# FrozenWolf-Cyber/Indic-CL-ASR

Hardware: AMD Instinct MI355X
Metric: utterances/sec (15 s @16 kHz) Conformer-M RNNT-CTC+EWC train step (higher is better)
Workload: dtype bf16; 1 GPU; BASELINE configs[1]: Conformer-medium (d=256, 16L, H=640) hybrid RNNT-CTC + EWC, bs=32/GPU x 15 s, bf16 projections, freeze_encoder_till=12, 22x257 heads, fused_batch_size=4; global_batch=32, parallelism=dp1

## Files before the change

### indic_cl_asr_amd/csrc/attention_flash_bwd.hip

```cpp
#include "attention_flash.h"
#include "partials.h"

namespace {

constexpr int FB_THREADS = 256;
constexpr int FB_ROWB = 128;
constexpr int FB_T64 = 64 * FB_ROWB;
constexpr int FB_PBUF = 128 * FB_ROWB;
constexpr int FB_SR_LD = 104;
constexpr int FB_SB_LD = 120;
constexpr int FB_Q_STRIP = 16 * (FB_SR_LD + FB_SB_LD) * 2;
constexpr int FB_Q_LDS = 2 * FB_T64 + FB_PBUF + 4 * FB_Q_STRIP;
constexpr int FB_S3_LD = 72;
constexpr int FB_KV_STAGE = 3 * FB_T64 + FB_PBUF + 512;
constexpr int FB_KV_LDS = FB_KV_STAGE + 4 * 16 * FB_S3_LD * 2;

struct FbArgs {
    const __bf16* qkv; const __bf16* pl; const float* bias_u; const float* bias_v; const int64_t* lens;
    const __bf16* ctx; const __bf16* dctx; const float* lse;
    __bf16* dqkv; __bf16* dBand; __bf16* QvHM; float* D; float* part;
    int B, T, H, dk, Rs, pad0; float scale; unsigned seed, thr; float keep_scale;
};

__device__ __forceinline__ void fb_lds_fence() {
    __builtin_amdgcn_fence(__ATOMIC_RELEASE, "wavefront");
    __builtin_amdgcn_wave_barrier();
    __builtin_amdgcn_fence(__ATOMIC_ACQUIRE, "wavefront");
}

__device__ __forceinline__ bf8 fb_tr_pair(const unsigned char* tile, int rowA, int rowB, int sl, int half) {
    const s4v lo = __builtin_amdgcn_ds_read_tr16_b64_v4i16(
        (__attribute__((address_space(3))) s4v*)(tile + rowA * FB_ROWB + ((sl ^ (rowA & 7)) * 16) + half * 8));
    const s4v hi = __builtin_amdgcn_ds_read_tr16_b64_v4i16(
        (__attribute__((address_space(3))) s4v*)(tile + rowB * FB_ROWB + ((sl ^ (rowB & 7)) * 16) + half * 8));
    union { s4v s[2]; bf8 v; } f;
    f.s[0] = lo; f.s[1] = hi;
    return f.v;
}

template <bool DK64>
__global__ __launch_bounds__(FB_THREADS, 2) void relpos_flash_bwd_q_kernel(FbArgs a) {
    extern __shared__ __attribute__((aligned(16))) unsigned char smem[];
    const int tid = threadIdx.x, lane = tid & 63, wave = tid >> 6;
    const int c = lane & 15, q4 = lane >> 4;
    const int T = a.T, H = a.H, dk = a.dk, d = H * dk, B = a.B;
    const int nqt = (T + 63) / 64;
    const int xcd = blockIdx.x & 7, slot_id = blockIdx.x >> 3;
    const int bh = xcd + 8 * (slot_id / nqt);
    if (bh >= B * H) return;
    const int qt = slot_id % nqt;
    const int h = bh % H, b = bh / H;
    int len = (int)a.lens[b];
    len = len < 0 ? 0 : (len > T ? T : len);
    const int I0 = qt * 64, iw = I0 + wave * 16, iq = iw + c;
    const int iqc = iq < T ? iq : T - 1;
    const bool qvalid = iq < len;
    float* part_row = a.part + (size_t)(b * nqt + qt) * (2 * d);

    bf8 Qu[2], Qv[2], dOa[2];
    float Drow = 0.f;
    {
        const __bf16* qrow = a.qkv + ((size_t)b * T + iqc) * (3 * d) + h * dk;
        const __bf16* orow = a.ctx + ((size_t)b * T + iqc) * d + h * dk;
        const __bf16* grow = a.dctx + ((size_t)b * T + iqc) * d + h * dk;
#pragma unroll
        for (int ks = 0; ks < 2; ++ks) {
            union { uint4 u; __bf16 e[8]; bf8 v; } q, o, g;
            q.u = fa_load_slot<DK64>(qrow, ks * 4 + q4, dk);
            o.u = fa_load_slot<DK64>(orow, ks * 4 + q4, dk);
            g.u = fa_load_slot<DK64>(grow, ks * 4 + q4, dk);
            dOa[ks] = g.v;
#pragma unroll
            for (int j = 0; j < 8; ++j) {
                const int e = ks * 32 + q4 * 8 + j;
                const float bu = (e < dk) ? a.bias_u[h * dk + e] : 0.f, bv = (e < dk) ? a.bias_v[h * dk + e] : 0.f;
                Qu[ks][j] = (__bf16)((float)q.e[j] + bu);
                Qv[ks][j] = (__bf16)((float)q.e[j] + bv);
                Drow += (float)g.e[j] * (float)o.e[j];
            }
            if (iq < T)
                *reinterpret_cast<bf8*>(a.QvHM + ((size_t)(h * B + b) * T + iq) * 64 + ks * 32 + q4 * 8) = Qv[ks];
        }
        Drow += __shfl_xor(Drow, 16, 64);
        Drow += __shfl_xor(Drow, 32, 64);
        if (!qvalid) Drow = 0.f;
        if (iq < T && q4 == 0) a.D[(size_t)bh * T + iq] = Drow;
    }
    const float lse_i = qvalid ? a.lse[(size_t)bh * T + iq] : 0.f;
    __bf16* dqrow = a.dqkv + ((size_t)b * T + iqc) * (3 * d) + h * dk;
    if (I0 >= len) {
        if (iq < T)
            for (int mt = 0; mt < 4; ++mt)
                if (mt * 16 + q4 * 4 < dk) *reinterpret_cast<uint2*>(dqrow + mt * 16 + q4 * 4) = make_uint2(0, 0);
        if (tid < 2 * dk) part_row[(tid / dk) * d + h * dk + (tid % dk)] = 0.f;
        return;
    }
    const unsigned char* sK = smem;
    const unsigned char* sV = smem + FB_T64;
    const unsigned char* sP = smem + 2 * FB_T64;
    unsigned char* sR = smem + 2 * FB_T64 + FB_PBUF + wave * FB_Q_STRIP;
    unsigned char* sB = sR + 16 * FB_SR_LD * 2;
    for (int i = lane; i < 16 * FB_SB_LD * 2 / 16; i += 64) reinterpret_cast<uint4*>(sB)[i] = make_uint4(0, 0, 0, 0);

    uint4 rk[2], rv[2], rp[4];
    const __bf16* kbase = a.qkv + (size_t)b * T * (3 * d) + d + h * dk;
    const __bf16* vbase = kbase + d;
    const __bf16* pbase = a.pl + h * dk;
#define FBQ_FETCH(t_)                                                                                         \
    do {                                                                                                      \
        const int j0_ = (t_) * 64;                                                                            \
        _Pragma("unroll") for (int i_ = 0; i_ < 2; ++i_) {                                                    \
            const int idx_ = tid + i_ * FB_THREADS, row_ = idx_ >> 3, sl_ = idx_ & 7;                         \
            int j_ = j0_ + row_; j_ = j_ < T ? j_ : T - 1;                                                    \
            rk[i_] = fa_load_slot<DK64>(kbase + (size_t)j_ * (3 * d), sl_, dk);                               \
            rv[i_] = fa_load_slot<DK64>(vbase + (size_t)j_ * (3 * d), sl_, dk);                               \
        }                                                                                                     \
        const int R0_ = T - 1 - I0 - 63 + j0_;                                                                \
        _Pragma("unroll") for (int i_ = 0; i_ < 4; ++i_) {                                                    \
            const int idx_ = tid + i_ * FB_THREADS, row_ = idx_ >> 3, sl_ = idx_ & 7;                         \
            int r_ = R0_ + row_; r_ = r_ < 0 ? 0 : (r_ > 2 * T - 2 ? 2 * T - 2 : r_);                         \
            rp[i_] = fa_load_slot<DK64>(pbase + (size_t)r_ * d, sl_, dk);                                     \
        }                                                                                                     \
    } while (0)
#define FBQ_COMMIT()                                                                                          \
    do {                                                                                                      \
        _Pragma("unroll") for (int i_ = 0; i_ < 2; ++i_) {                                                    \
            const int idx_ = tid + i_ * FB_THREADS, row_ = idx_ >> 3, sl_ = idx_ & 7;                         \
            const int off_ = row_ * FB_ROWB + ((sl_ ^ (row_ & 7)) * 16);                                      \
            *reinterpret_cast<uint4*>(smem + off_) = rk[i_];                                                  \
            *reinterpret_cast<uint4*>(smem + FB_T64 + off_) = rv[i_];                                         \
        }                                                                                                     \
        _Pragma("unroll") for (int i_ = 0; i_ < 4; ++i_) {                                                    \
            const int idx_ = tid + i_ * FB_THREADS, row_ = idx_ >> 3, sl_ = idx_ & 7;                         \
            *reinterpret_cast<uint4*>(smem + 2 * FB_T64 + row_ * FB_ROWB + ((sl_ ^ (row_ & 7)) * 16)) = rp[i_]; \
        }                                                                                                     \
    } while (0)

    const int nkt = (len + 63) / 64;
    FBQ_FETCH(0);
    FBQ_COMMIT();
    __syncthreads();

    f4 dQu[4], dQv[4];
#pragma unroll
    for (int mt = 0; mt < 4; ++mt) { dQu[mt] = (f4){0.f, 0.f, 0.f, 0.f}; dQv[mt] = (f4){0.f, 0.f, 0.f, 0.f}; }
    const int frow = lane >> 2, fch = (lane & 3) * 2;
    __bf16* brow = a.dBand + ((size_t)(h * B + b) * T + (iw + frow < T ? iw + frow : T - 1)) * a.Rs;
    const bool fvalid = iw + frow < T;
    const int pw0 = (3 - wave) * 16;

    for (int t = 0; t < nkt; ++t) {
        if (t + 1 < nkt) FBQ_FETCH(t + 1);
        const int j0 = t * 64;
        {
            f4 R[5];
#pragma unroll
            for (int rt = 0; rt < 5; ++rt) {
                R[rt] = (f4){0.f, 0.f, 0.f, 0.f};
                const int row = pw0 + rt * 16 + c;
#pragma unroll
                for (int ks = 0; ks < 2; ++ks) {
                    const bf8 pf = *reinterpret_cast<const bf8*>(sP + row * FB_ROWB + (((ks * 4 + q4) ^ (row & 7)) * 16));
                    R[rt] = __builtin_amdgcn_mfma_f32_16x16x32_bf16(pf, Qv[ks], R[rt], 0, 0, 0);
                }
            }
#pragma unroll
            for (int rt = 0; rt < 5; ++rt)
#pragma unroll
                for (int r = 0; r < 4; ++r)
                    *reinterpret_cast<__bf16*>(sR + (c * FB_SR_LD + rt * 16 + q4 * 4 + r + c + 1) * 2) = (__bf16)R[rt][r];
        }
        f4 S[4], dP[4];
#pragma unroll
        for (int jt = 0; jt < 4; ++jt) {
            S[jt] = (f4){0.f, 0.f, 0.f, 0.f};
            dP[jt] = (f4){0.f, 0.f, 0.f, 0.f};
            const int row = jt * 16 + c;
#pragma unroll
            for (int ks = 0; ks < 2; ++ks) {
                const int off = row * FB_ROWB + (((ks * 4 + q4) ^ (row & 7)) * 16);
                const bf8 kf = *reinterpret_cast<const bf8*>(sK + off);
                const bf8 vf = *reinterpret_cast<const bf8*>(sV + off);
                S[jt] = __builtin_amdgcn_mfma_f32_16x16x32_bf16(kf, Qu[ks], S[jt], 0, 0, 0);
                dP[jt] = __builtin_amdgcn_mfma_f32_16x16x32_bf16(vf, dOa[ks], dP[jt], 0, 0, 0);
            }
        }
        fb_lds_fence();
        bf8 dSf[2];
#pragma unroll
        for (int jt = 0; jt < 4; ++jt) {
            union { uint2 u; __bf16 e[4]; } bd;
            bd.u = *reinterpret_cast<const uint2*>(sR + (c * FB_SR_LD + jt * 16 + q4 * 4 + 16) * 2);
            unsigned rnd4 = 0;
            if (a.thr > 0) rnd4 = fa_keep_rand4(a.seed, bh, T, iq, (j0 + jt * 16 + q4 * 4) >> 2);
#pragma unroll
            for (int r = 0; r < 4; ++r) {
                const int j = j0 + jt * 16 + q4 * 4 + r;
                const float s = (S[jt][r] + (float)bd.e[r]) * a.scale;
                const float p = (qvalid && j < len) ? __expf(s - lse_i) : 0.f;
                float g = dP[jt][r];
                if (a.thr > 0) g = (((rnd4 >> (8 * r)) & 0xFFu) >= a.thr) ? g * a.keep_scale : 0.f;
                const float ds = p * (g - Drow) * a.scale;
                const __bf16 dsb = (__bf16)ds;
                dSf[jt >> 1][(jt & 1) * 4 + r] = dsb;
                S[jt][r] = (float)dsb;
            }
        }
#pragma unroll
        for (int kk = 0; kk < 2; ++kk)
#pragma unroll
            for (int mt = 0; mt < 4; ++mt) {
                const int qq = c >> 2, p = c & 3;
                const int rowA = kk * 32 + q4 * 4 + qq;
                const bf8 kf = fb_tr_pair(sK, rowA, rowA + 16, mt * 2 + (p >> 1), p & 1);
                dQu[mt] = __builtin_amdgcn_mfma_f32_16x16x32_bf16(kf, dSf[kk], dQu[mt], 0, 0, 0);
            }
        for (int i = lane; i < 16 * 12; i += 64) {
            const int row = i / 12, ch = i - row * 12;
            *reinterpret_cast<uint4*>(sB + (row * FB_SB_LD + ch * 8) * 2) = make_uint4(0, 0, 0, 0);
        }
        fb_lds_fence();
#pragma unroll
        for (int jt = 0; jt < 4; ++jt)
#pragma unroll
            for (int r = 0; r < 4; ++r)
                *reinterpret_cast<__bf16*>(sB + (c * FB_SB_LD + jt * 16 + q4 * 4 + r + 15 - c) * 2) = (__bf16)S[jt][r];
        fb_lds_fence();
#pragma unroll
        for (int kk = 0; kk < 3; ++kk) {
            const bf8 bfrag = *reinterpret_cast<const bf8*>(sB + (c * FB_SB_LD + kk * 32 + q4 * 8) * 2);
#pragma unroll
            for (int mt = 0; mt < 4; ++mt) {
                const int qq = c >> 2, p = c & 3;
                int rowA = pw0 + kk * 32 + q4 * 8 + qq, rowB = rowA + 4;
                rowA = rowA < 127 ? rowA : 127; rowB = rowB < 127 ? rowB : 127;
                const bf8 pf = fb_tr_pair(sP, rowA, rowB, mt * 2 + (p >> 1), p & 1);
                dQv[mt] = __builtin_amdgcn_mfma_f32_16x16x32_bf16(pf, bfrag, dQv[mt], 0, 0, 0);
            }
        }
        {
            uint4 v0 = *reinterpret_cast<const uint4*>(sB + (frow * FB_SB_LD + fch * 8) * 2);
            uint4 v1 = *reinterpret_cast<const uint4*>(sB + (frow * FB_SB_LD + fch * 8 + 8) * 2);
            if ((lane & 3) == 0) {
                const uint4 c0 = *reinterpret_cast<const uint4*>(sB + (frow * FB_SB_LD + 96) * 2);
                const uint4 c1 = *reinterpret_cast<const uint4*>(sB + (frow * FB_SB_LD + 104) * 2);
                v0.x |= c0.x; v0.y |= c0.y; v0.z |= c0.z; v0.w |= c0.w;
                v1.x |= c1.x; v1.y |= c1.y; v1.z |= c1.z; v1.w |= c1.w;
                const uint4 n0 = *reinterpret_cast<const uint4*>(sB + (frow * FB_SB_LD + 64) * 2);
                const uint4 n1 = *reinterpret_cast<const uint4*>(sB + (frow * FB_SB_LD + 72) * 2);
                *reinterpret_cast<uint4*>(sB + (frow * FB_SB_LD + 96) * 2) = n0;
                *reinterpret_cast<uint4*>(sB + (frow * FB_SB_LD + 104) * 2) = n1;
            }
            if (fvalid) {
                const int gcol = T - 16 - iw + j0 + a.pad0 + fch * 8;
                if (gcol >= 0) *reinterpret_cast<uint4*>(brow + gcol) = v0;
                if (gcol + 8 >= 0) *reinterpret_cast<uint4*>(brow + gcol + 8) = v1;
            }
        }
        __syncthreads();
        if (t + 1 < nkt) {
            FBQ_COMMIT();
            __syncthreads();
        }
    }
#undef FBQ_FETCH
#undef FBQ_COMMIT
    fb_lds_fence();
    if ((lane & 3) == 0 && fvalid) {
        const int gcol = T - 16 - iw + (nkt - 1) * 64 + a.pad0 + 64;
        *reinterpret_cast<uint4*>(brow + gcol) = *reinterpret_cast<const uint4*>(sB + (frow * FB_SB_LD + 96) * 2);
        *reinterpret_cast<uint4*>(brow + gcol + 8) = *reinterpret_cast<const uint4*>(sB + (frow * FB_SB_LD + 104) * 2);
    }
    if (iq < T) {
#pragma unroll
        for (int mt = 0; mt < 4; ++mt) {
            if (mt * 16 + q4 * 4 < dk) {
                union { uint2 u; __bf16 e[4]; } o;
#pragma unroll
                for (int r = 0; r < 4; ++r) o.e[r] = (__bf16)(dQu[mt][r] + dQv[mt][r]);
                *reinterpret_cast<uint2*>(dqrow + mt * 16 + q4 * 4) = o.u;
            }
        }
    }
    float* red = reinterpret_cast<float*>(smem);
#pragma unroll
    for (int mt = 0; mt < 4; ++mt)
#pragma unroll
        for (int r = 0; r < 4; ++r) {
            float su = dQu[mt][r], sv = dQv[mt][r];
#pragma unroll
            for (int o = 1; o < 16; o <<= 1) { su += __shfl_xor(su, o, 64); sv += __shfl_xor(sv, o, 64); }
            if (c == 0) {
                red[(wave * 2 + 0) * 64 + mt * 16 + q4 * 4 + r] = su;
                red[(wave * 2 + 1) * 64 + mt * 16 + q4 * 4 + r] = sv;
            }
        }
    __syncthreads();
    if (tid < 2 * dk) {
        const int which = tid / dk, e = tid % dk;
        part_row[which * d + h * dk + e] = (red[(0 * 2 + which) * 64 + e] + red[(1 * 2 + which) * 64 + e]) +
                                           (red[(2 * 2 + which) * 64 + e] + red[(3 * 2 + which) * 64 + e]);
    }
}

template <bool DK64>
__global__ __launch_bounds__(FB_THREADS, 2) void relpos_flash_bwd_kv_kernel(FbArgs a) {
    extern __shared__ __attribute__((aligned(16))) unsigned char smem[];
    const int tid = threadIdx.x, lane = tid & 63, wave = tid >> 6;
    const int c = lane & 15, q4 = lane >> 4;
    const int T = a.T, H = a.H, dk = a.dk, d = H * dk, B = a.B;
    const int nkt = (T + 63) / 64;
    const int xcd = blockIdx.x & 7, slot_id = blockIdx.x >> 3;
    const int bh = xcd + 8 * (slot_id / nkt);
    if (bh >= B * H) return;
    const int kt = slot_id % nkt;
    const int h = bh % H, b = bh / H;
    int len = (int)a.lens[b];
    len = len < 0 ? 0 : (len > T ? T : len);
    const int J0 = kt * 64, jw = J0 + wave * 16, j = jw + c;
    const int jc = j < T ? j : T - 1;
    const bool kvalid = j < len;
    __bf16* dkrow = a.dqkv + ((size_t)b * T + jc) * (3 * d) + d + h * dk;
    __bf16* dvrow = dkrow + d;
    if (J0 >= len) {
        if (j < T)
            for (int mt = 0; mt < 4; ++mt)
                if (mt * 16 + q4 * 4 < dk) {
                    *reinterpret_cast<uint2*>(dkrow + mt * 16 + q4 * 4) = make_uint2(0, 0);
                    *reinterpret_cast<uint2*>(dvrow + mt * 16 + q4 * 4) = make_uint2(0, 0);
                }
        return;
    }
    bf8 Kf[2], Vf[2];
    {
        const __bf16* krow = a.qkv + ((size_t)b * T + jc) * (3 * d) + d + h * dk;
#pragma unroll
        for (int ks = 0; ks < 2; ++ks) {
            union { uint4 u; bf8 v; } k, v;
            k.u = fa_load_slot<DK64>(krow, ks * 4 + q4, dk);
            v.u = fa_load_slot<DK64>(krow + d, ks * 4 + q4, dk);
            Kf[ks] = k.v; Vf[ks] = v.v;
        }
    }
    const unsigned char* sQu = smem;
    const unsigned char* sQv = smem + FB_T64;
    const unsigned char* sdO = smem + 2 * FB_T64;
    const unsigned char* sP = smem + 3 * FB_T64;
    const float* sL = reinterpret_cast<const float*>(smem + 3 * FB_T64 + FB_PBUF);
    unsigned char* s3 = smem + FB_KV_STAGE + wave * (16 * FB_S3_LD * 2);

    float bu[8], bv[8];
    {
        const int sl = tid & 7;
#pragma unroll
        for (int e = 0; e < 8; ++e) {
            const int ee = sl * 8 + e;
            bu[e] = (ee < dk) ? a.bias_u[h * dk + ee] : 0.f;
            bv[e] = (ee < dk) ? a.bias_v[h * dk + ee] : 0.f;
        }
    }
    uint4 rq[2], rg[2], rp[4];
    float rl = 0.f;
    const __bf16* qbase = a.qkv + (size_t)b * T * (3 * d) + h * dk;
    const __bf16* gbase = a.dctx + (size_t)b * T * d + h * dk;
    const __bf16* pbase = a.pl + h * dk;
#define FBK_FETCH(t_)                                                                                         \
    do {                                                                                                      \
        const int i0_ = (t_) * 64;                                                                            \
        _Pragma("unroll") for (int i_ = 0; i_ < 2; ++i_) {                                                    \
            const int idx_ = tid + i_ * FB_THREADS, row_ = idx_ >> 3, sl_ = idx_ & 7;                         \
            int q_ = i0_ + row_; q_ = q_ < T ? q_ : T - 1;                                                    \
            rq[i_] = fa_load_slot<DK64>(qbase + (size_t)q_ * (3 * d), sl_, dk);                               \
            rg[i_] = fa_load_slot<DK64>(gbase + (size_t)q_ * d, sl_, dk);                                     \
        }                                                                                                     \
        const int R0_ = T - 1 - i0_ - 63 + J0;                                                                \
        _Pragma("unroll") for (int i_ = 0; i_ < 4; ++i_) {                                                    \
            const int idx_ = tid + i_ * FB_THREADS, row_ = idx_ >> 3, sl_ = idx_ & 7;                         \
            int r_ = R0_ + row_; r_ = r_ < 0 ? 0 : (r_ > 2 * T - 2 ? 2 * T - 2 : r_);                         \
            rp[i_] = fa_load_slot<DK64>(pbase + (size_t)r_ * d, sl_, dk);                                     \
        }                                                                                                     \
        if (tid < 128) {                                                                                      \
            int q_ = i0_ + (tid & 63); q_ = q_ < T ? q_ : T - 1;                                              \
            rl = (tid < 64 ? a.lse : a.D)[(size_t)bh * T + q_];                                               \
        }                                                                                                     \
    } while (0)
#define FBK_COMMIT()                                                                                          \
    do {                                                                                                      \
        _Pragma("unroll") for (int i_ = 0; i_ < 2; ++i_) {                                                    \
            const int idx_ = tid + i_ * FB_THREADS, row_ = idx_ >> 3, sl_ = idx_ & 7;                         \
            const int off_ = row_ * FB_ROWB + ((sl_ ^ (row_ & 7)) * 16);                                      \
            union { uint4 u; __bf16 e[8]; } q_, u_, v_;                                                       \
            q_.u = rq[i_];                                                                                    \
            _Pragma("unroll") for (int e_ = 0; e_ < 8; ++e_) {                                                \
                u_.e[e_] = (__bf16)((float)q_.e[e_] + bu[e_]);                                                \
                v_.e[e_] = (__bf16)((float)q_.e[e_] + bv[e_]);                                                \
            }                                                                                                 \
            *reinterpret_cast<uint4*>(smem + off_) = u_.u;                                                    \
            *reinterpret_cast<uint4*>(smem + FB_T64 + off_) = v_.u;                                           \
            *reinterpret_cast<uint4*>(smem + 2 * FB_T64 + off_) = rg[i_];                                     \
        }                                                                                                     \
        _Pragma("unroll") for (int i_ = 0; i_ < 4; ++i_) {                                                    \
            const int idx_ = tid + i_ * FB_THREADS, row_ = idx_ >> 3, sl_ = idx_ & 7;                         \
            *reinterpret_cast<uint4*>(smem + 3 * FB_T64 + row_ * FB_ROWB + ((sl_ ^ (row_ & 7)) * 16)) = rp[i_]; \
        }                                                                                                     \
        if (tid < 128) reinterpret_cast<float*>(smem + 3 * FB_T64 + FB_PBUF)[tid] = rl;                       \
    } while (0)

    const int nqt = (len + 63) / 64;
    FBK_FETCH(0);
    FBK_COMMIT();
    __syncthreads();

    f4 dK[4], dV[4];
#pragma unroll
    for (int mt = 0; mt < 4; ++mt) { dK[mt] = (f4){0.f, 0.f, 0.f, 0.f}; dV[mt] = (f4){0.f, 0.f, 0.f, 0.f}; }

    for (int t = 0; t < nqt; ++t) {
        if (t + 1 < nqt) FBK_FETCH(t + 1);
        const int I0 = t * 64;
#pragma unroll
        for (int it = 0; it < 4; ++it) {
            f4 XA = (f4){0.f, 0.f, 0.f, 0.f}, XB = (f4){0.f, 0.f, 0.f, 0.f};
            const int qrow = it * 16 + c;
            const int n0 = 48 - 16 * it + 16 * wave;
            const int pa = n0 + c, pb = n0 + 16 + c;
#pragma unroll
            for (int ks = 0; ks < 2; ++ks) {
                const bf8 qf = *reinterpret_cast<const bf8*>(sQv + qrow * FB_ROWB + (((ks * 4 + q4) ^ (qrow & 7)) * 16));
                const bf8 fa = *reinterpret_cast<const bf8*>(sP + pa * FB_ROWB + (((ks * 4 + q4) ^ (pa & 7)) * 16));
                const bf8 fb = *reinterpret_cast<const bf8*>(sP + pb * FB_ROWB + (((ks * 4 + q4) ^ (pb & 7)) * 16));
                XA = __builtin_amdgcn_mfma_f32_16x16x32_bf16(qf, fa, XA, 0, 0, 0);
                XB = __builtin_amdgcn_mfma_f32_16x16x32_bf16(qf, fb, XB, 0, 0, 0);
            }
#pragma unroll
            for (int r = 0; r < 4; ++r) {
                const int m = q4 * 4 + r;
                const int keyA = c - 15 + m, keyB = c + m + 1;
                if (keyA >= 0) *reinterpret_cast<__bf16*>(s3 + (keyA * FB_S3_LD + it * 16 + m) * 2) = (__bf16)XA[r];
                if (keyB <= 15) *reinterpret_cast<__bf16*>(s3 + (keyB * FB_S3_LD + it * 16 + m) * 2) = (__bf16)XB[r];
            }
        }
        f4 S[4], dP[4];
#pragma unroll
        for (int it = 0; it < 4; ++it) {
            S[it] = (f4){0.f, 0.f, 0.f, 0.f};
            dP[it] = (f4){0.f, 0.f, 0.f, 0.f};
            const int row = it * 16 + c;
#pragma unroll
            for (int ks = 0; ks < 2; ++ks) {
                const int off = row * FB_ROWB + (((ks * 4 + q4) ^ (row & 7)) * 16);
                const bf8 qf = *reinterpret_cast<const bf8*>(sQu + off);
                const bf8 gf = *reinterpret_cast<const bf8*>(sdO + off);
                S[it] = __builtin_amdgcn_mfma_f32_16x16x32_bf16(qf, Kf[ks], S[it], 0, 0, 0);
                dP[it] = __builtin_amdgcn_mfma_f32_16x16x32_bf16(gf, Vf[ks], dP[it], 0, 0, 0);
            }
        }
        fb_lds_fence();
        bf8 Pdf[2], dSf[2];
#pragma unroll
        for (int it = 0; it < 4; ++it) {
            union { uint2 u; __bf16 e[4]; } bd;
            bd.u = *reinterpret_cast<const uint2*>(s3 + (c * FB_S3_LD + it * 16 + q4 * 4) * 2);
            const float4 ls = *reinterpret_cast<const float4*>(sL + it * 16 + q4 * 4);
            const float4 dd = *reinterpret_cast<const float4*>(sL + 64 + it * 16 + q4 * 4);
            const float lsv[4] = {ls.x, ls.y, ls.z, ls.w}, ddv[4] = {dd.x, dd.y, dd.z, dd.w};
#pragma unroll
            for (int r = 0; r < 4; ++r) {
                const int i = I0 + it * 16 + q4 * 4 + r;
                const float s = (S[it][r] + (float)bd.e[r]) * a.scale;
                const float p = (kvalid && i < len) ? __expf(s - lsv[r]) : 0.f;
                float g = dP[it][r], pd = p;
                if (a.thr > 0) {
                    const unsigned rnd = (fa_keep_rand4(a.seed, bh, T, i, j >> 2) >> (8 * (j & 3))) & 0xFFu;
                    const bool keep = rnd >= a.thr;
                    g = keep ? g * a.keep_scale : 0.f;
                    pd = keep ? p * a.keep_scale : 0.f;
                }
                const float ds = p * (g - ddv[r]) * a.scale;
                Pdf[it >> 1][(it & 1) * 4 + r] = (__bf16)pd;
                dSf[it >> 1][(it & 1) * 4 + r] = (__bf16)ds;
            }
        }
#pragma unroll
        for (int kk = 0; kk < 2; ++kk)
#pragma unroll
            for (int mt = 0; mt < 4; ++mt) {
                const int qq = c >> 2, p = c & 3;
                const int rowA = kk * 32 + q4 * 4 + qq;
                const bf8 gf = fb_tr_pair(sdO, rowA, rowA + 16, mt * 2 + (p >> 1), p & 1);
                const bf8 qf = fb_tr_pair(sQu, rowA, rowA + 16, mt * 2 + (p >> 1), p & 1);
                dV[mt] = __builtin_amdgcn_mfma_f32_16x16x32_bf16(gf, Pdf[kk], dV[mt], 0, 0, 0);
                dK[mt] = __builtin_amdgcn_mfma_f32_16x16x32_bf16(qf, dSf[kk], dK[mt], 0, 0, 0);
            }
        __syncthreads();
        if (t + 1 < nqt) {
            FBK_COMMIT();
            __syncthreads();
        }
    }
#undef FBK_FETCH
#undef FBK_COMMIT
    if (j < T) {
#pragma unroll
        for (int mt = 0; mt < 4; ++mt) {
            if (mt * 16 + q4 * 4 < dk) {
                union { uint2 u; __bf16 e[4]; } ok, ov;
#pragma unroll
                for (int r = 0; r < 4; ++r) { ok.e[r] = (__bf16)dK[mt][r]; ov.e[r] = (__bf16)dV[mt][r]; }
                *reinterpret_cast<uint2*>(dkrow + mt * 16 + q4 * 4) = ok.u;
                *reinterpret_cast<uint2*>(dvrow + mt * 16 + q4 * 4) = ov.u;
            }
        }
    }
}

__global__ __launch_bounds__(256) void fb_dpos_pack_kernel(const float* __restrict__ dpos, int H, int Rs, int pad0, int R, int dk,
                                                           int rows, __bf16* __restrict__ out) {
    const int d = H * dk, q = dk / 4;
    const int64_t total = (int64_t)rows * H * q;
    for (int64_t i = (int64_t)blockIdx.x * 256 + threadIdx.x; i < total; i += (int64_t)gridDim.x * 256) {
        const int e4 = (int)(i % q);
        const int h = (int)((i / q) % H);
        const int r = (int)(i / ((int64_t)q * H));
        union { uint2 u; __bf16 e[4]; } o;
        o.u = make_uint2(0, 0);
        if (r < R) {
            const float4 v = *reinterpret_cast<const float4*>(dpos + (size_t)h * ((size_t)Rs * 64 + Rs) + (size_t)(pad0 + r) * 64 + e4 * 4);
            o.e[0] = (__bf16)v.x; o.e[1] = (__bf16)v.y; o.e[2] = (__bf16)v.z; o.e[3] = (__bf16)v.w;
        }
        *reinterpret_cast<uint2*>(out + (size_t)r * d + h * dk + e4 * 4) = o.u;
    }
}

}

extern "C" int ia_relpos_attention_flash_bwd_dims(int T, int* Rs, int* pad0) {
    if (T <= 0 || !Rs || !pad0) return IA_INVALID_VALUE;
    const int p0 = (8 - ((T + 8 * 16 - 16) % 8)) % 8;
    const int nkt = (T + 63) / 64;
    *pad0 = p0;
    *Rs = (T - 16 + p0 + 64 * nkt + 16 + 7) / 8 * 8;
    if (*Rs < p0 + 2 * T - 1) *Rs = (p0 + 2 * T - 1 + 7) / 8 * 8;
    return IA_OK;
}

namespace {
struct FbWs { int64_t part, D, dpos, tn, total; };
inline FbWs fb_ws_layout(int B, int T, int H, int dk) {
    int rs, p0;
    ia_relpos_attention_flash_bwd_dims(T, &rs, &p0);
    FbWs w;
    auto up = [](int64_t x) { return (x + 63) / 64 * 64; };
    w.part = 0;
    w.D = up((int64_t)B * ((T + 63) / 64) * 2 * H * dk);
    w.dpos = w.D + up((int64_t)B * H * T);
    w.tn = w.dpos + up((int64_t)H * ((int64_t)rs * 64 + rs));
    {
        ia_tn_problem pr[8];
        const int nh = H < 8 ? H : 8;
        for (int i = 0; i < nh; ++i) pr[i] = ia_tn_problem{nullptr, nullptr, nullptr, nullptr, rs, 64, B * T, rs, 64};
        w.total = w.tn + up(ia_gemm_tn_grouped_scratch_elems(pr, nh));
    }
    return w;
}
}

extern "C" int64_t ia_relpos_attention_flash_bwd_ws_elems(int B, int T, int H, int dk) {
    if (B <= 0 || T <= 0 || H <= 0 || dk <= 0) return 0;
    return fb_ws_layout(B, T, H, dk).total;
}

extern "C" int ia_relpos_attention_flash_bwd(const void* qkv, const void* pos_proj, const float* bias_u, const float* bias_v,
                                             const int64_t* lens, const void* ctx, const void* dctx, const float* lse, int B,
                                             int T, int H, int dk, float dropout_p, unsigned seed, void* dqkv, void* dpl,
                                             int pl_rows, float* dbias_u, float* dbias_v, void* dBand, void* QvHM, float* ws,
                                             ia_stream_t stream) {
    if (!qkv || !pos_proj || !bias_u || !bias_v || !lens || !ctx || !dctx || !lse || !dqkv || !dpl || !dBand || !QvHM || !ws ||
        !dbias_u || !dbias_v || B <= 0 || T <= 0 || H <= 0 || pl_rows < 2 * T - 1)
        return IA_INVALID_VALUE;
    if (!ia_relpos_attention_flash_supported(T, dk)) return IA_UNSUPPORTED;
    if (dropout_p < 0.f || dropout_p >= 1.f) return IA_INVALID_VALUE;
    if (!ia_is_aligned(qkv, 16) || !ia_is_aligned(pos_proj, 16) || !ia_is_aligned(ctx, 8) || !ia_is_aligned(dctx, 8) ||
        !ia_is_aligned(dqkv, 8) || !ia_is_aligned(dBand, 16) || !ia_is_aligned(QvHM, 16) || !ia_is_aligned(ws, 16) ||
        !ia_is_aligned(dpl, 8))
        return IA_INVALID_VALUE;
    const FbWs w = fb_ws_layout(B, T, H, dk);
    FbArgs a;
    a.qkv = (const __bf16*)qkv; a.pl = (const __bf16*)pos_proj; a.bias_u = bias_u; a.bias_v = bias_v; a.lens = lens;
    a.ctx = (const __bf16*)ctx; a.dctx = (const __bf16*)dctx; a.lse = lse; a.dqkv = (__bf16*)dqkv; a.dBand = (__bf16*)dBand;
    a.QvHM = (__bf16*)QvHM; a.D = ws + w.D; a.part = ws + w.part; a.B = B; a.T = T; a.H = H; a.dk = dk;
    int rs, p0;
    ia_relpos_attention_flash_bwd_dims(T, &rs, &p0);
    a.Rs = rs; a.pad0 = p0;
    a.scale = 1.f / sqrtf((float)dk); a.seed = seed;
    const ia_dropout_t drop = ia_dropout_rule(dropout_p);
    a.thr = drop.thr; a.keep_scale = drop.keep_scale;
    hipStream_t st = (hipStream_t)stream;
    if (hipMemsetAsync(dBand, 0, (size_t)H * B * T * rs * sizeof(__bf16), st) != hipSuccess) return IA_LAUNCH_FAILED;
    const int nt = (T + 63) / 64;
    const int grid = 8 * ((B * H + 7) / 8) * nt;
    const bool full = (dk == 64);
    if (full) {
        IA_SET_MAX_LDS_ONCE((relpos_flash_bwd_q_kernel<true>), FB_Q_LDS);
        hipLaunchKernelGGL((relpos_flash_bwd_q_kernel<true>), dim3(grid), dim3(FB_THREADS), FB_Q_LDS, st, a);
    } else {
        IA_SET_MAX_LDS_ONCE((relpos_flash_bwd_q_kernel<false>), FB_Q_LDS);
        hipLaunchKernelGGL((relpos_flash_bwd_q_kernel<false>), dim3(grid), dim3(FB_THREADS), FB_Q_LDS, st, a);
    }
    IA_RETURN_IF_LAUNCH_FAILED();
    if (full) {
        IA_SET_MAX_LDS_ONCE((relpos_flash_bwd_kv_kernel<true>), FB_KV_LDS);
        hipLaunchKernelGGL((relpos_flash_bwd_kv_kernel<true>), dim3(grid), dim3(FB_THREADS), FB_KV_LDS, st, a);
    } else {
        IA_SET_MAX_LDS_ONCE((relpos_flash_bwd_kv_kernel<false>), FB_KV_LDS);
        hipLaunchKernelGGL((relpos_flash_bwd_kv_kernel<false>), dim3(grid), dim3(FB_THREADS), FB_KV_LDS, st, a);
    }
    IA_RETURN_IF_LAUNCH_FAILED();
    ia_partials_finish(a.part, B * nt, 2 * H * dk, H * dk, dbias_u, dbias_v, st);
    IA_RETURN_IF_LAUNCH_FAILED();
    float* dpos = ws + w.dpos;
    for (int h0 = 0; h0 < H; h0 += 8) {
        ia_tn_problem pr[8];
        const int nh = H - h0 < 8 ? H - h0 : 8;
        for (int i = 0; i < nh; ++i) {
            const int h = h0 + i;
            float* o = dpos + (size_t)h * ((size_t)rs * 64 + rs);
            pr[i] = ia_tn_problem{(const __bf16*)dBand + (size_t)h * B * T * rs, (const __bf16*)QvHM + (size_t)h * B * T * 64, o, nullptr,
                                  rs, 64, B * T, rs, 64};
        }
        const int rc = ia_gemm_tn_bf16_grouped(pr, nh, ws + w.tn, stream);
        if (rc != IA_OK) return rc;
    }
    const int64_t items = (int64_t)pl_rows * H * (dk / 4);
    const int64_t blocks = (items + 255) / 256;
    hipLaunchKernelGGL(fb_dpos_pack_kernel, dim3((unsigned)(blocks < 4096 ? blocks : 4096)), dim3(256), 0, st, (const float*)dpos, H, rs,
                       p0, 2 * T - 1, dk, pl_rows, (__bf16*)dpl);
    IA_RETURN_IF_LAUNCH_FAILED();
    return IA_OK;
}
```

### indic_cl_asr_amd/csrc/block_train.hip

```cpp
#include <hip/hip_bf16.h>
#include <hip/hip_runtime.h>

#include <cstdint>

#include <cstdlib>

#include "ia_common.h"

namespace {

inline size_t up256(size_t x) { return (x + 255) / 256 * 256; }

#define IA_TRY(call)                  \
    do {                              \
        const int rc_ = (call);       \
        if (rc_ != IA_OK) return rc_; \
    } while (0)

__global__ __launch_bounds__(256) void transpose_bf16_kernel(const unsigned short* __restrict__ in, int rows, int cols,
                                                             unsigned short* __restrict__ out) {
    __shared__ unsigned short tile[64][72];
    const int tiles_c = (cols + 63) / 64;
    const int tr = blockIdx.x / tiles_c, tc = blockIdx.x - tr * tiles_c;
    const int r0 = tr * 64, c0 = tc * 64;
    for (int i = threadIdx.x; i < 64 * 8; i += 256) {
        const int r = i >> 3, v = i & 7;
        uint4 x = make_uint4(0, 0, 0, 0);
        if (r0 + r < rows && c0 + v * 8 < cols) x = *reinterpret_cast<const uint4*>(in + (size_t)(r0 + r) * cols + c0 + v * 8);
        *reinterpret_cast<uint4*>(&tile[r][v * 8]) = x;
    }
    __syncthreads();
    for (int i = threadIdx.x; i < 64 * 8; i += 256) {
        const int c = i >> 3, v = i & 7;
        if (c0 + c < cols && r0 + v * 8 < rows) {
            union { uint4 u; unsigned short h[8]; } o;
#pragma unroll
            for (int j = 0; j < 8; ++j) o.h[j] = tile[v * 8 + j][c];
            *reinterpret_cast<uint4*>(out + (size_t)(c0 + c) * rows + r0 + v * 8) = o.u;
        }
    }
}

int transpose_bf16(const void* in, int rows, int cols, void* out, hipStream_t st) {
    if (rows % 8 != 0 || cols % 8 != 0) return IA_UNSUPPORTED;
    const int grid = ((rows + 63) / 64) * ((cols + 63) / 64);
    hipLaunchKernelGGL(transpose_bf16_kernel, dim3(grid), dim3(256), 0, st, (const unsigned short*)in, rows, cols, (unsigned short*)out);
    IA_RETURN_IF_LAUNCH_FAILED();
    return IA_OK;
}

struct TrJob { const unsigned short* in; unsigned short* out; int rows, cols, tile_begin, tiles_c; };
struct TrJobs { TrJob j[8]; int count; };
__global__ __launch_bounds__(256) void transpose_bf16_multi_kernel(TrJobs jobs) {
    __shared__ unsigned short tile[64][72];
    int ji = 0;
#pragma unroll
    for (int i = 1; i < 8; ++i)
        if (i < jobs.count && (int)blockIdx.x >= jobs.j[i].tile_begin) ji = i;
    const TrJob& J = jobs.j[ji];
    const int local = blockIdx.x - J.tile_begin;
    const int tr = local / J.tiles_c, tc = local - tr * J.tiles_c;
    const int r0 = tr * 64, c0 = tc * 64, rows = J.rows, cols = J.cols;
    for (int i = threadIdx.x; i < 64 * 8; i += 256) {
        const int r = i >> 3, v = i & 7;
        uint4 x = make_uint4(0, 0, 0, 0);
        if (r0 + r < rows && c0 + v * 8 < cols) x = *reinterpret_cast<const uint4*>(J.in + (size_t)(r0 + r) * cols + c0 + v * 8);
        *reinterpret_cast<uint4*>(&tile[r][v * 8]) = x;
    }
    __syncthreads();
    for (int i = threadIdx.x; i < 64 * 8; i += 256) {
        const int c = i >> 3, v = i & 7;
        if (c0 + c < cols && r0 + v * 8 < rows) {
            union { uint4 u; unsigned short h[8]; } o;
#pragma unroll
            for (int j = 0; j < 8; ++j) o.h[j] = tile[v * 8 + j][c];
            *reinterpret_cast<uint4*>(J.out + (size_t)(c0 + c) * rows + r0 + v * 8) = o.u;
        }
    }
}
struct TrList { TrJobs jobs; int tiles; };
inline void tr_add(TrList* l, const void* in, int rows, int cols, void* out) {
    TrJob& J = l->jobs.j[l->jobs.count++];
    J.in = (const unsigned short*)in; J.out = (unsigned short*)out; J.rows = rows; J.cols = cols;
    J.tile_begin = l->tiles; J.tiles_c = (cols + 63) / 64;
    l->tiles += ((rows + 63) / 64) * J.tiles_c;
}
int tr_launch(const TrList& l, hipStream_t st) {
    for (int i = 0; i < l.jobs.count; ++i)
        if (l.jobs.j[i].rows % 8 != 0 || l.jobs.j[i].cols % 8 != 0) return IA_UNSUPPORTED;
    hipLaunchKernelGGL(transpose_bf16_multi_kernel, dim3(l.tiles), dim3(256), 0, st, l.jobs);
    IA_RETURN_IF_LAUNCH_FAILED();
    return IA_OK;
}

struct AddRow { float* dst; const float* src; int64_t n; };
__global__ __launch_bounds__(256) void multi_add_kernel(const AddRow* __restrict__ table, int rows) {
    for (int k = blockIdx.y; k < rows; k += gridDim.y) {
        const AddRow r = table[k];
        const int64_t n4 = ((reinterpret_cast<uintptr_t>(r.dst) | reinterpret_cast<uintptr_t>(r.src)) & 15) ? 0 : (r.n >> 2);
        for (int64_t i = (int64_t)blockIdx.x * 256 + threadIdx.x; i < n4; i += (int64_t)gridDim.x * 256) {
            float4 a = reinterpret_cast<float4*>(r.dst)[i];
            const float4 b = reinterpret_cast<const float4*>(r.src)[i];
            a.x += b.x; a.y += b.y; a.z += b.z; a.w += b.w;
            reinterpret_cast<float4*>(r.dst)[i] = a;
        }
        for (int64_t i = (n4 << 2) + (int64_t)blockIdx.x * 256 + threadIdx.x; i < r.n; i += (int64_t)gridDim.x * 256) r.dst[i] += r.src[i];
    }
}

struct BwdWs {
    size_t dxa, dxb, dB, dB1, dB2, dB3, dh, dhp, dy, dc3, dz, dG, dc2, dctx, wt, scr, total;
};

size_t max3(size_t a, size_t b, size_t c) { return a > b ? (a > c ? a : c) : (b > c ? b : c); }

BwdWs bwd_ws(int B, int T, int d, int d_ff, int ksz) {
    const size_t N = (size_t)B * T;
    BwdWs w;
    size_t o = 0;
    w.dxa = o;  o = up256(o + N * d * 4);
    w.dxb = o;  o = up256(o + N * d * 4);
    w.dB = o;   o = up256(o + N * d * 2);
    w.dB1 = o;  o = up256(o + N * d * 2);
    w.dB2 = o;  o = up256(o + N * d * 2);
    w.dB3 = o;  o = up256(o + N * d * 2);
    w.dh = o;   o = up256(o + N * d_ff * 2);
    w.dhp = o;  o = up256(o + N * d_ff * 2);
    w.dy = o;   o = up256(o + N * d * 2);
    w.dc3 = o;  o = up256(o + N * d * 2);
    w.dz = o;   o = up256(o + N * d * 4);
    w.dG = o;   o = up256(o + (size_t)5 * (size_t)ia_layernorm_bwd_scratch_elems((int)N, d) * 4);
    w.dc2 = o;  o = up256(o + N * 2 * d * 2);
    w.dctx = o; o = up256(o + N * d * 2);
    w.wt = o;   o = up256(o + ((size_t)4 * d_ff * d + (size_t)7 * d * d) * 2);
    size_t scr = (size_t)ia_layernorm_bwd_scratch_elems((int)N, d);
    const int shapes[5][2] = {{d, d_ff}, {d_ff, d}, {d, d}, {2 * d, d}, {3 * d, d}};
    for (int i = 0; i < 5; ++i) {
        const size_t e = (size_t)ia_gemm_tn_scratch_elems((int)N, shapes[i][0], shapes[i][1]);
        scr = e > scr ? e : scr;
    }
    scr = max3(scr, (size_t)ia_bn_silu_bwd_scratch_elems((int64_t)N, d), (size_t)ia_dwconv_scratch_elems(B, T, d, ksz));
    {
        const ia_tn_problem ga[5] = {{nullptr, nullptr, nullptr, nullptr, d, d_ff, (int)N, d, d_ff},
                                     {nullptr, nullptr, nullptr, nullptr, d_ff, d, (int)N, d_ff, d},
                                     {nullptr, nullptr, nullptr, nullptr, d, d, (int)N, d, d},
                                     {nullptr, nullptr, nullptr, nullptr, 2 * d, d, (int)N, 2 * d, d},
                                     {nullptr, nullptr, nullptr, nullptr, d, d, (int)N, d, d}};
        const ia_tn_problem gb[4] = {{nullptr, nullptr, nullptr, nullptr, 3 * d, d, (int)N, 3 * d, d},
                                     {nullptr, nullptr, nullptr, nullptr, d, d, (int)(N > (size_t)64 * 512 ? N : (size_t)64 * 512), d, d},
                                     {nullptr, nullptr, nullptr, nullptr, d, d_ff, (int)N, d, d_ff},
                                     {nullptr, nullptr, nullptr, nullptr, d_ff, d, (int)N, d_ff, d}};
        scr = max3(scr, (size_t)ia_gemm_tn_grouped_scratch_elems(ga, 5), (size_t)ia_gemm_tn_grouped_scratch_elems(gb, 4));
        scr = max3(scr, (size_t)ia_gemm_tn_grouped_scratch_elems(gb, 2), (size_t)ia_gemm_tn_grouped_scratch_elems(gb + 2, 2));
        ia_tn_problem gall[9];
        for (int i = 0; i < 5; ++i) gall[i] = ga[i];
        for (int i = 0; i < 4; ++i) gall[5 + i] = gb[i];
        scr = scr > (size_t)ia_gemm_tn_grouped_scratch_elems(gall, 9) ? scr : (size_t)ia_gemm_tn_grouped_scratch_elems(gall, 9);
    }
    w.scr = o;  o = up256(o + scr * 4);
    w.total = o;
    return w;
}

int linear_bwd(const void* dY, const void* X, const void* W, int M, int n, int k, void* dX, float* dW, float* db, void* wt,
               float* scr, ia_stream_t stream) {
    if (dX) {
        IA_TRY(transpose_bf16(W, n, k, wt, (hipStream_t)stream));
        IA_TRY(ia_gemm_bf16(dY, n, wt, n, M, k, n, nullptr, 0, 0.f, 0, 1.f, nullptr, 0, nullptr, 0, dX, k, stream));
    }
    return ia_gemm_tn_bf16(dY, n, X, k, M, n, k, dW, db, scr, stream);
}

bool tn_grouping_enabled() {
    static const bool on = [] { const char* e = getenv("IA_TN_GROUPED"); return !(e && e[0] == '0'); }();
    return on;
}
int flush_group(const ia_tn_problem* grp, int ngrp, float* scr, ia_stream_t stream) {
    if (tn_grouping_enabled()) return ia_gemm_tn_bf16_grouped(grp, ngrp, scr, stream);
    for (int i = 0; i < ngrp; ++i)
        IA_TRY(ia_gemm_tn_bf16(grp[i].dY, grp[i].ldy, grp[i].X, grp[i].ldx, grp[i].M, grp[i].n, grp[i].k, grp[i].dW, grp[i].db, scr, stream));
    return IA_OK;
}
int linear_bwd_deferred(const void* dY, const void* X, const void* W, int M, int n, int k, void* dX, float* dW, float* db, const void* wt,
                        ia_tn_problem* grp, int* ngrp, ia_stream_t stream) {
    (void)W;
    if (dX) IA_TRY(ia_gemm_bf16(dY, n, wt, n, M, k, n, nullptr, 0, 0.f, 0, 1.f, nullptr, 0, nullptr, 0, dX, k, stream));
    grp[*ngrp] = ia_tn_problem{dY, X, dW, db, n, k, M, n, k};
    ++*ngrp;
    return IA_OK;
}

struct SideCtx {
    hipStream_t s = nullptr;
    hipEvent_t ev[8] = {};
    bool ok = false, tried = false;
    bool a_pending = false;
};
SideCtx* side_ctx() {
    static SideCtx ctx[16];
    const char* e = getenv("IA_WGRAD_SIDE");
    if (!(e && e[0] == '1')) return nullptr;
    int dev = 0;
    if (hipGetDevice(&dev) != hipSuccess || dev < 0 || dev >= 16) return nullptr;
    SideCtx& c = ctx[dev];
    if (!c.tried) {
        c.tried = true;
        bool ok = hipStreamCreateWithFlags(&c.s, hipStreamNonBlocking) == hipSuccess;
        for (int i = 0; ok && i < 8; ++i) ok = hipEventCreateWithFlags(&c.ev[i], hipEventDisableTiming) == hipSuccess;
        c.ok = ok;
    }
    return c.ok ? &c : nullptr;
}
struct PendingGroup { ia_tn_problem grp[8]; int n = 0; const void* ws = nullptr; };
PendingGroup* pending_group() {
    static PendingGroup pg[16];
    int dev = 0;
    if (hipGetDevice(&dev) != hipSuccess || dev < 0 || dev >= 16) return nullptr;
    return &pg[dev];
}
bool merged_wgrads() {
    const char* e = getenv("IA_TN_MERGE");
    return !(e && e[0] == '0') && tn_grouping_enabled();
}

int stream_after(hipStream_t from, hipStream_t to, hipEvent_t ev) {
    if (hipEventRecord(ev, from) != hipSuccess || hipStreamWaitEvent(to, ev, 0) != hipSuccess) return IA_LAUNCH_FAILED;
    return IA_OK;
}

}

extern "C" size_t ia_conformer_block_bwd_ws_bytes(int B, int T, int d, int d_ff, int ksz) {
    if (B <= 0 || T <= 0 || d <= 0 || d_ff <= 0 || ksz <= 0) return 0;
    return bwd_ws(B, T, d, d_ff, ksz).total;
}

extern "C" int ia_conformer_block_supported(int d, int d_ff, int H, int ksz, int T) {
    if (d <= 0 || H <= 0 || d % H != 0) return 0;
    const int dk = d / H;
    return (d % 8 == 0 && d <= 1024 && d_ff % 8 == 0 && ksz <= 31 && (ksz & 1) == 1 && dk <= 64 && dk % 4 == 0 && T >= 1) ? 1 : 0;
}

extern "C" int ia_conformer_block_fwd(const ia_block_params* Lp, const float* x0, const void* pos_emb, int pos_rows,
                                      const int64_t* lens, int B, int T, unsigned seed, const ia_block_saved* Sp, float* out,
                                      float* dw_scratch, ia_stream_t stream) {
    return ia_conformer_block_fwd_phase(Lp, x0, pos_emb, pos_rows, lens, B, T, seed, Sp, out, dw_scratch, 0, stream);
}

extern "C" int ia_conformer_block_fwd_phase(const ia_block_params* Lp, const float* x0, const void* pos_emb, int pos_rows,
                                            const int64_t* lens, int B, int T, unsigned seed, const ia_block_saved* Sp,
                                            float* out, float* dw_scratch, int phase, ia_stream_t stream) {
    if (phase < 0 || phase > 2) return IA_INVALID_VALUE;
    if (!Lp || !x0 || !pos_emb || !lens || !Sp || !out || !dw_scratch || B <= 0 || T <= 0) return IA_INVALID_VALUE;
    const ia_block_params& L = *Lp;
    const ia_block_saved& S = *Sp;
    const int d = L.d, d_ff = L.d_ff, H = L.n_heads, dk = d / (H > 0 ? H : 1), ksz = L.ksz, N = B * T;
    if (!ia_conformer_block_supported(d, d_ff, H, ksz, T) || pos_rows < 2 * T - 1) return IA_UNSUPPORTED;
    const float p = L.p_drop, pff = L.p_ff, patt = L.p_att;
    if (phase != 2) {
    IA_TRY(ia_layernorm(x0, d, N, d, L.ln_ff1_g, L.ln_ff1_b, L.ln_eps, nullptr, 0, nullptr, nullptr, S.y1, d, stream));
    IA_TRY(ia_gemm_bf16_ex(S.y1, d, L.w_ff1a, d, N, d_ff, d, L.b_ff1a, 1, pff, seed + 1, 1.f, nullptr, 0, nullptr, 0, S.h1, d_ff,
                           S.h1p, d_ff, nullptr, 0, stream));
    IA_TRY(ia_gemm_bf16(S.h1, d_ff, L.w_ff1b, d_ff, N, d, d_ff, L.b_ff1b, 0, p, seed + 2, L.fc_factor, x0, d, S.x1, d, nullptr, 0, stream));
    IA_TRY(ia_layernorm(S.x1, d, N, d, L.ln_att_g, L.ln_att_b, L.ln_eps, nullptr, 0, nullptr, nullptr, S.y2, d, stream));
    IA_TRY(ia_gemm_bf16(S.y2, d, L.w_qkv, d, N, 3 * d, d, L.b_qkv, 0, 0.f, 0, 1.f, nullptr, 0, nullptr, 0, S.qkv, 3 * d, stream));
    IA_TRY(ia_gemm_bf16(pos_emb, d, L.w_pos, d, pos_rows, d, d, nullptr, 0, 0.f, 0, 1.f, nullptr, 0, nullptr, 0, S.pl, d, stream));
    IA_TRY(ia_relpos_attention_flash_lse(S.qkv, S.pl, L.pos_u, L.pos_v, lens, B, T, H, dk, patt, seed + 7, S.ctxv, S.lse, stream));
    IA_TRY(ia_gemm_bf16(S.ctxv, d, L.w_out, d, N, d, d, L.b_out, 0, p, seed + 3, 1.f, S.x1, d, S.x2, d, nullptr, 0, stream));
    IA_TRY(ia_layernorm(S.x2, d, N, d, L.ln_conv_g, L.ln_conv_b, L.ln_eps, nullptr, 0, nullptr, nullptr, S.y3, d, stream));
    IA_TRY(ia_gemm_bf16(S.y3, d, L.w_pw1, d, N, 2 * d, d, L.b_pw1, 0, 0.f, 0, 1.f, nullptr, 0, nullptr, 0, S.c2, 2 * d, stream));
    IA_TRY(ia_glu_dwconv(S.c2, lens, B, T, d, ksz, L.dw_w, L.dw_b, S.z, S.sums, S.sums + d, dw_scratch, stream));
    }
    if (phase == 1) return IA_OK;
    const bool synced = phase == 2;
    if (ia_gemm_bnsilu_supported(d)) {
        IA_TRY(ia_gemm_bnsilu_bf16_keep(S.z, d, N, S.sums, S.sums + d, L.bn_g, L.bn_b, synced ? nullptr : L.bn_rm,
                                        synced ? nullptr : L.bn_rv, synced ? nullptr : L.bn_nbt, L.bn_momentum, L.bn_eps, 1, L.w_pw2,
                                        d, N, d, d, L.b_pw2, p, seed + 4, 1.f, S.x2, d, S.x3, d, nullptr, 0, nullptr, S.c3, d, stream));
    } else {
        IA_TRY(ia_bn_silu(S.z, N, d, S.sums, S.sums + d, L.bn_g, L.bn_b, synced ? nullptr : L.bn_rm, synced ? nullptr : L.bn_rv,
                          synced ? nullptr : L.bn_nbt, L.bn_momentum, L.bn_eps, 1, S.c3, stream));
        IA_TRY(ia_gemm_bf16(S.c3, d, L.w_pw2, d, N, d, d, L.b_pw2, 0, p, seed + 4, 1.f, S.x2, d, S.x3, d, nullptr, 0, stream));
    }
    IA_TRY(ia_layernorm(S.x3, d, N, d, L.ln_ff2_g, L.ln_ff2_b, L.ln_eps, nullptr, 0, nullptr, nullptr, S.y4, d, stream));
    IA_TRY(ia_gemm_bf16_ex(S.y4, d, L.w_ff2a, d, N, d_ff, d, L.b_ff2a, 1, pff, seed + 5, 1.f, nullptr, 0, nullptr, 0, S.h4, d_ff,
                           S.h4p, d_ff, nullptr, 0, stream));
    IA_TRY(ia_gemm_bf16(S.h4, d_ff, L.w_ff2b, d_ff, N, d, d_ff, L.b_ff2b, 0, p, seed + 6, L.fc_factor, S.x3, d, S.x4, d, nullptr, 0, stream));
    return ia_layernorm(S.x4, d, N, d, L.ln_out_g, L.ln_out_b, L.ln_eps, out, d, nullptr, nullptr, nullptr, 0, stream);
}

extern "C" int ia_conformer_block_bwd_a(const ia_block_params* Lp, const ia_block_saved* Sp, const ia_block_grads* Gp,
                                        const float* dout, const int64_t* lens, int B, int T, unsigned seed, void* workspace,
                                        size_t workspace_bytes, float** dx2_out, void** dctx_out, ia_stream_t stream) {
    return ia_conformer_block_bwd_a_phase(Lp, Sp, Gp, dout, lens, B, T, seed, workspace, workspace_bytes, dx2_out, dctx_out, 0, nullptr,
                                          stream);
}

extern "C" int ia_conformer_block_bwd_a_phase(const ia_block_params* Lp, const ia_block_saved* Sp, const ia_block_grads* Gp,
                                              const float* dout, const int64_t* lens, int B, int T, unsigned seed,
                                              void* workspace, size_t workspace_bytes, float** dx2_out, void** dctx_out,
                                              int phase, const float* bn_S12, ia_stream_t stream) {
    if (phase < 0 || phase > 2 || (phase == 2 && !bn_S12)) return IA_INVALID_VALUE;
    if (!Lp || !Sp || !Gp || !dout || !lens || !workspace || !dx2_out || !dctx_out || B <= 0 || T <= 0) return IA_INVALID_VALUE;
    const ia_block_params& L = *Lp;
    const ia_block_saved& S = *Sp;
    const ia_block_grads& G = *Gp;
    const int d = L.d, d_ff = L.d_ff, ksz = L.ksz, N = B * T;
    const BwdWs w = bwd_ws(B, T, d, d_ff, ksz);
    if (workspace_bytes < w.total) return IA_WORKSPACE_TOO_SMALL;
    char* ws = (char*)workspace;
    float *dxa = (float*)(ws + w.dxa), *dxb = (float*)(ws + w.dxb), *dz = (float*)(ws + w.dz), *scr = (float*)(ws + w.scr);
    float* lnp = (float*)(ws + w.dG);
    const size_t lnp_set = (size_t)ia_layernorm_bwd_scratch_elems(N, d);
    void *dB = ws + w.dB, *dB1 = ws + w.dB1, *dB2 = ws + w.dB2, *dhp = ws + w.dhp, *dy = ws + w.dy, *dc3 = ws + w.dc3, *dc2 = ws + w.dc2,
         *dctx = ws + w.dctx, *wt = ws + w.wt;
    const float p = L.p_drop, pff = L.p_ff;
    ia_tn_problem grp[8];
    int ngrp = 0;
    char* wtb = (char*)wt;
    void *wt_ff2b = wtb, *wt_ff2a = wtb + (size_t)d * d_ff * 2, *wt_pw2 = wtb + (size_t)2 * d * d_ff * 2,
         *wt_pw1 = wtb + ((size_t)2 * d * d_ff + (size_t)d * d) * 2, *wt_out = wtb + ((size_t)2 * d * d_ff + (size_t)3 * d * d) * 2;
    if (phase != 2) {
        TrList tl{};
        tr_add(&tl, L.w_ff2b, d, d_ff, wt_ff2b); tr_add(&tl, L.w_ff2a, d_ff, d, wt_ff2a); tr_add(&tl, L.w_pw2, d, d, wt_pw2);
        tr_add(&tl, L.w_pw1, 2 * d, d, wt_pw1); tr_add(&tl, L.w_out, d, d, wt_out);
        IA_TRY(tr_launch(tl, (hipStream_t)stream));
    }
    if (phase != 2) {
    IA_TRY(ia_layernorm_bwd_drop(S.x4, d, dout, nullptr, d, N, d, L.ln_out_g, L.ln_eps, nullptr, dxa, d, nullptr, nullptr,
                                 L.fc_factor, p, seed + 6, dB, d, lnp + 0 * lnp_set, stream));
    IA_TRY(ia_gemm_bf16_ex(dB, d, wt_ff2b, d, N, d_ff, d, nullptr, 3, pff, seed + 5, 1.f, nullptr, 0, nullptr, 0, dhp, d_ff, nullptr, 0,
                           S.h4p, d_ff, stream));
    IA_TRY(linear_bwd_deferred(dB, S.h4, L.w_ff2b, N, d, d_ff, nullptr, G.w_ff2b, G.b_ff2b, wt_ff2b, grp, &ngrp, stream));
    IA_TRY(linear_bwd_deferred(dhp, S.y4, L.w_ff2a, N, d_ff, d, dy, G.w_ff2a, G.b_ff2a, wt_ff2a, grp, &ngrp, stream));
    IA_TRY(ia_layernorm_bwd_drop(S.x3, d, nullptr, dy, d, N, d, L.ln_ff2_g, L.ln_eps, dxa, dxb, d, nullptr, nullptr, 1.f, p,
                                 seed + 4, dB1, d, lnp + 1 * lnp_set, stream));
    IA_TRY(linear_bwd_deferred(dB1, S.c3, L.w_pw2, N, d, d, dc3, G.w_pw2, G.b_pw2, wt_pw2, grp, &ngrp, stream));
    if (phase == 0)
        IA_TRY(ia_bn_silu_bwd(S.z, dc3, N, d, S.sums, S.sums + d, L.bn_g, L.bn_b, L.bn_eps, G.bn_b, G.bn_g, dz, scr, stream));
    else
        IA_TRY(ia_bn_silu_bwd_reduce(S.z, dc3, N, d, S.sums, S.sums + d, L.bn_g, L.bn_b, L.bn_eps, G.bn_b, G.bn_g, scr, stream));
    }
    if (phase == 1) {
        IA_TRY(flush_group(grp, ngrp, scr, stream));
        return IA_OK;
    }
    if (phase == 2)
        IA_TRY(ia_bn_silu_bwd_apply(S.z, dc3, N, d, S.sums, S.sums + d, L.bn_g, L.bn_b, L.bn_eps, bn_S12, bn_S12 + d, dz, stream));
    IA_TRY(ia_dwconv_glu_bwd(dz, S.c2, lens, B, T, d, ksz, L.dw_w, dc2, stream));
    SideCtx* side = phase == 0 ? side_ctx() : nullptr;
    hipStream_t main = (hipStream_t)stream;
    if (side) {
        IA_TRY(stream_after(main, side->s, side->ev[0]));
        IA_TRY(ia_dwconv_glu_wgrad(S.c2, lens, dz, B, T, d, ksz, G.dw_w, G.dw_b, scr, (ia_stream_t)side->s));
    } else {
        IA_TRY(ia_dwconv_glu_wgrad(S.c2, lens, dz, B, T, d, ksz, G.dw_w, G.dw_b, scr, stream));
    }
    IA_TRY(linear_bwd_deferred(dc2, S.y3, L.w_pw1, N, 2 * d, d, dy, G.w_pw1, G.b_pw1, wt_pw1, grp, &ngrp, stream));
    IA_TRY(ia_layernorm_bwd_drop(S.x2, d, nullptr, dy, d, N, d, L.ln_conv_g, L.ln_eps, dxb, dxa, d, nullptr, nullptr, 1.f, p,
                                 seed + 3, dB2, d, lnp + 2 * lnp_set, stream));
    IA_TRY(linear_bwd_deferred(dB2, S.ctxv, L.w_out, N, d, d, dctx, G.w_out, G.b_out, wt_out, grp, &ngrp, stream));
    if (side) {
        IA_TRY(stream_after(main, side->s, side->ev[1]));
        IA_TRY(flush_group(grp, ngrp, scr, (ia_stream_t)side->s));
        if (hipEventRecord(side->ev[2], side->s) != hipSuccess) return IA_LAUNCH_FAILED;
        side->a_pending = true;
    } else if (phase == 0 && merged_wgrads() && pending_group()) {
        PendingGroup* pg = pending_group();
        for (int i = 0; i < ngrp; ++i) pg->grp[i] = grp[i];
        pg->n = ngrp; pg->ws = workspace;
    } else {
        IA_TRY(flush_group(grp, ngrp, scr, stream));
    }
    *dx2_out = dxa;
    *dctx_out = dctx;
    return IA_OK;
}

extern "C" int ia_conformer_block_bwd_b(const ia_block_params* Lp, const ia_block_saved* Sp, const ia_block_grads* Gp,
                                        const float* x0, const void* pos_emb, int pos_rows, const void* dqkv, const void* dpl,
                                        int B, int T, unsigned seed, void* workspace, size_t workspace_bytes, float* dx0,
                                        const void* add_table, int n_add, ia_stream_t stream) {
    if (!Lp || !Sp || !Gp || !x0 || !pos_emb || !dqkv || !dpl || !workspace || !dx0 || B <= 0 || T <= 0) return IA_INVALID_VALUE;
    const ia_block_params& L = *Lp;
    const ia_block_saved& S = *Sp;
    const ia_block_grads& G = *Gp;
    const int d = L.d, d_ff = L.d_ff, ksz = L.ksz, N = B * T;
    const BwdWs w = bwd_ws(B, T, d, d_ff, ksz);
    if (workspace_bytes < w.total) return IA_WORKSPACE_TOO_SMALL;
    char* ws = (char*)workspace;
    float *dxa = (float*)(ws + w.dxa), *dxb = (float*)(ws + w.dxb), *scr = (float*)(ws + w.scr);
    float* lnp = (float*)(ws + w.dG);
    const size_t lnp_set = (size_t)ia_layernorm_bwd_scratch_elems(N, d);
    PendingGroup* pg = pending_group();
    const bool carried = pg && pg->n > 0 && pg->ws == workspace;
    void *dB = ws + (carried ? w.dB3 : w.dB), *dhp = ws + (carried ? w.dh : w.dhp), *dy = ws + w.dy, *wt = ws + w.wt;
    const float p = L.p_drop, pff = L.p_ff;
    ia_tn_problem grp[12];
    int ngrp = 0;
    if (carried) {
        for (int i = 0; i < pg->n; ++i) grp[ngrp++] = pg->grp[i];
        pg->n = 0;
    }
    char* wtb = (char*)wt + ((size_t)2 * d * d_ff + (size_t)4 * d * d) * 2;
    void *wt_qkv = wtb, *wt_ff1b = wtb + (size_t)3 * d * d * 2, *wt_ff1a = wtb + ((size_t)3 * d * d + (size_t)d * d_ff) * 2;
    {
        TrList tl{};
        tr_add(&tl, L.w_qkv, 3 * d, d, wt_qkv); tr_add(&tl, L.w_ff1b, d, d_ff, wt_ff1b); tr_add(&tl, L.w_ff1a, d_ff, d, wt_ff1a);
        IA_TRY(tr_launch(tl, (hipStream_t)stream));
    }
    SideCtx* side = carried ? nullptr : side_ctx();
    hipStream_t main = (hipStream_t)stream;
    IA_TRY(linear_bwd_deferred(dqkv, S.y2, L.w_qkv, N, 3 * d, d, dy, G.w_qkv, G.b_qkv, wt_qkv, grp, &ngrp, stream));
    grp[ngrp++] = ia_tn_problem{dpl, pos_emb, G.w_pos, nullptr, d, d, pos_rows, d, d};
    if (side) {
        IA_TRY(stream_after(main, side->s, side->ev[3]));
        IA_TRY(flush_group(grp, ngrp, scr, (ia_stream_t)side->s));
        ngrp = 0;
        if (side->a_pending) {
            if (hipStreamWaitEvent(main, side->ev[2], 0) != hipSuccess) return IA_LAUNCH_FAILED;
            side->a_pending = false;
        }
    }
    IA_TRY(ia_layernorm_bwd_drop(S.x1, d, nullptr, dy, d, N, d, L.ln_att_g, L.ln_eps, dxa, dxb, d, nullptr, nullptr, L.fc_factor,
                                 p, seed + 2, dB, d, lnp + 3 * lnp_set, stream));
    IA_TRY(ia_gemm_bf16_ex(dB, d, wt_ff1b, d, N, d_ff, d, nullptr, 3, pff, seed + 1, 1.f, nullptr, 0, nullptr, 0, dhp, d_ff, nullptr, 0,
                           S.h1p, d_ff, stream));
    IA_TRY(linear_bwd_deferred(dB, S.h1, L.w_ff1b, N, d, d_ff, nullptr, G.w_ff1b, G.b_ff1b, wt_ff1b, grp, &ngrp, stream));
    if (side) {
        grp[ngrp++] = ia_tn_problem{dhp, S.y1, G.w_ff1a, G.b_ff1a, d_ff, d, N, d_ff, d};
        IA_TRY(stream_after(main, side->s, side->ev[4]));
        IA_TRY(flush_group(grp, ngrp, scr, (ia_stream_t)side->s));
        ngrp = 0;
        IA_TRY(ia_gemm_bf16(dhp, d_ff, wt_ff1a, d_ff, N, d, d_ff, nullptr, 0, 0.f, 0, 1.f, nullptr, 0, nullptr, 0, dy, d, stream));
    } else {
        IA_TRY(linear_bwd_deferred(dhp, S.y1, L.w_ff1a, N, d_ff, d, dy, G.w_ff1a, G.b_ff1a, wt_ff1a, grp, &ngrp, stream));
    }
    IA_TRY(ia_layernorm_bwd(x0, d, nullptr, dy, d, N, d, L.ln_ff1_g, L.ln_eps, dxb, dx0, d, nullptr, nullptr, lnp + 4 * lnp_set, stream));
    if (side) {
        IA_TRY(stream_after(main, side->s, side->ev[5]));
        stream = (ia_stream_t)side->s;
    } else {
        IA_TRY(flush_group(grp, ngrp, scr, stream));
    }
    {
        const int rows = ia_layernorm_bwd_partial_rows(N);
        const ia_finish_job jobs[5] = {{lnp + 0 * lnp_set, rows, 2 * d, d, G.ln_out_g, G.ln_out_b},
                                       {lnp + 1 * lnp_set, rows, 2 * d, d, G.ln_ff2_g, G.ln_ff2_b},
                                       {lnp + 2 * lnp_set, rows, 2 * d, d, G.ln_conv_g, G.ln_conv_b},
                                       {lnp + 3 * lnp_set, rows, 2 * d, d, G.ln_att_g, G.ln_att_b},
                                       {lnp + 4 * lnp_set, rows, 2 * d, d, G.ln_ff1_g, G.ln_ff1_b}};
        IA_TRY(ia_partials_finish_multi(jobs, 5, stream));
    }
    if (add_table && n_add > 0) {
        hipLaunchKernelGGL(multi_add_kernel, dim3(64, n_add < 64 ? n_add : 64), dim3(256), 0, (hipStream_t)stream,
                           (const AddRow*)add_table, n_add);
        IA_RETURN_IF_LAUNCH_FAILED();
    }
    if (side) IA_TRY(stream_after(side->s, main, side->ev[6]));
    return IA_OK;
}
```

### indic_cl_asr_amd/csrc/dwconv.hip

```cpp
#include <hip/hip_bf16.h>

#include <cstdint>
#include <cstdlib>

#include "ia_common.h"
#include "indicasr.h"
#include "partials.h"

namespace {

constexpr int DW_TT = 16;
constexpr int DW_TB = 4 * DW_TT;

template <int KMAX>
__device__ __forceinline__ void load_taps(float (&wt)[KMAX], const float* __restrict__ w, int c, int ksz, int flip) {
    const int off = (KMAX - 1) / 2 - (ksz - 1) / 2;
#pragma unroll
    for (int jj = 0; jj < KMAX; ++jj) {
        const int j = jj - off;
        wt[jj] = (j >= 0 && j < ksz) ? w[c * ksz + (flip ? ksz - 1 - j : j)] : 0.f;
    }
}

template <int KMAX, int GLU>
__global__ __launch_bounds__(256) void dwconv_fwd_kernel(const void* __restrict__ xin, const int64_t* __restrict__ lens, int B,
                                                         int T, int d, int ksz, const float* __restrict__ w,
                                                         const float* __restrict__ bias, int flip, float* __restrict__ y,
                                                         float* __restrict__ part, long long* __restrict__ acc,
                                                         const __bf16* __restrict__ c2 = nullptr, __bf16* __restrict__ dc2 = nullptr) {
    constexpr int HM = (KMAX - 1) / 2, WIN = DW_TT + KMAX - 1;
    const int lane = threadIdx.x & 63, wv = threadIdx.x >> 6;
    const int ntb = (T + DW_TB - 1) / DW_TB;
    const int b = blockIdx.x / ntb, t0 = (blockIdx.x - b * ntb) * DW_TB + wv * DW_TT;
    const int c = blockIdx.y * 64 + lane;
    const bool cok = c < d;
    const int cc = cok ? c : d - 1;
    int tmax = T;
    if (GLU == 1 || GLU == 2) { const int len = (int)lens[b]; tmax = len < T ? len : T; }
    float wt[KMAX];
    load_taps<KMAX>(wt, w, cc, ksz, flip);
    float win[WIN];
#pragma unroll
    for (int r = 0; r < WIN; ++r) {
        const int t = t0 - HM + r;
        const bool ok = t >= 0 && t < tmax;
        const int tt = t < 0 ? 0 : (t >= T ? T - 1 : t);
        float v;
        if (GLU == 1) {
            const __bf16* p = reinterpret_cast<const __bf16*>(xin) + ((size_t)b * T + tt) * (2 * d);
            const float a = (float)p[cc], gate = (float)p[d + cc];
            v = a * ia_sigmoid_fast(gate);
        } else if (GLU == 2) {
            v = (float)reinterpret_cast<const __bf16*>(xin)[((size_t)b * T + tt) * d + cc];
        } else {
            v = reinterpret_cast<const float*>(xin)[((size_t)b * T + tt) * d + cc];
        }
        win[r] = ok ? v : 0.f;
    }
    const float bb = bias ? bias[cc] : 0.f;
    float s = 0.f, s2 = 0.f;
#pragma unroll
    for (int i = 0; i < DW_TT; ++i) {
        float acc = bb;
#pragma unroll
        for (int jj = 0; jj < KMAX; ++jj) acc += wt[jj] * win[i + jj];
        const int t = t0 + i;
        if (t < T && cok) {
            if (GLU == 3) {
                const size_t row = (size_t)b * T + t;
                const float av = (float)c2[row * 2 * d + c], gv = (float)c2[row * 2 * d + d + c];
                const float sg = ia_sigmoid_fast(gv);
                const float dg = (t < (int)lens[b]) ? acc : 0.f;
                dc2[row * 2 * d + c] = (__bf16)(dg * sg);
                dc2[row * 2 * d + d + c] = (__bf16)(dg * av * sg * (1.f - sg));
            } else {
                y[((size_t)b * T + t) * d + c] = acc;
                s += acc; s2 += acc * acc;
            }
        }
    }
    if (GLU == 1 || GLU == 2) {
        __shared__ float red[4][2][64];
        red[wv][0][lane] = s; red[wv][1][lane] = s2;
        __syncthreads();
        if (wv == 0 && cok) {
            const float t1 = (red[0][0][lane] + red[1][0][lane]) + (red[2][0][lane] + red[3][0][lane]);
            const float t2 = (red[0][1][lane] + red[1][1][lane]) + (red[2][1][lane] + red[3][1][lane]);
            if (acc) {
                long long* mine = acc + (size_t)(blockIdx.x & (IA_BN_ACC_COPIES - 1)) * 2 * d;
                atomicAdd(reinterpret_cast<unsigned long long*>(mine + c), (unsigned long long)__float2ll_rn(t1 * 16777216.f));
                atomicAdd(reinterpret_cast<unsigned long long*>(mine + d + c), (unsigned long long)__float2ll_rn(t2 * 16777216.f));
            } else {
                part[(size_t)blockIdx.x * 2 * d + c] = t1;
                part[(size_t)blockIdx.x * 2 * d + d + c] = t2;
            }
        }
    }
}

template <int KMAX, bool XGLU>
__global__ __launch_bounds__(256) void dwconv_wgrad_kernel(const float* __restrict__ x, const float* __restrict__ dy, int B,
                                                           int T, int d, int nsplit, float* __restrict__ part,
                                                           const __bf16* __restrict__ c2 = nullptr,
                                                           const int64_t* __restrict__ lens = nullptr) {
    constexpr int HM = (KMAX - 1) / 2, WIN = DW_TT + KMAX - 1;
    const int lane = threadIdx.x & 63, wv = threadIdx.x >> 6;
    const int b = blockIdx.x / nsplit, sp = blockIdx.x - b * nsplit;
    const int per = (((T + nsplit - 1) / nsplit + DW_TT - 1) / DW_TT) * DW_TT;
    const int ts = sp * per, te = (ts + per < T) ? ts + per : T;
    const int c = blockIdx.y * 64 + lane;
    const bool cok = c < d;
    const int cc = cok ? c : d - 1;
    float acc[KMAX];
#pragma unroll
    for (int jj = 0; jj < KMAX; ++jj) acc[jj] = 0.f;
    float sb = 0.f;
    int tlen = T;
    if constexpr (XGLU) { const int len = (int)lens[b]; tlen = len < T ? len : T; }
    for (int t0 = ts + wv * DW_TT; t0 < te; t0 += 4 * DW_TT) {
        float g[DW_TT], win[WIN];
#pragma unroll
        for (int i = 0; i < DW_TT; ++i) {
            const int t = t0 + i;
            const float v = dy[((size_t)b * T + (t < T ? t : T - 1)) * d + cc];
            g[i] = (t < te) ? v : 0.f;
        }
#pragma unroll
        for (int r = 0; r < WIN; ++r) {
            const int t = t0 - HM + r;
            const int tt = t < 0 ? 0 : (t >= T ? T - 1 : t);
            if constexpr (XGLU) {
                const size_t row = (size_t)b * T + tt;
                const float av = (float)c2[row * 2 * d + cc], gv = (float)c2[row * 2 * d + d + cc];
                win[r] = (t >= 0 && t < tlen) ? av * ia_sigmoid_fast(gv) : 0.f;
            } else {
                const float v = x[((size_t)b * T + tt) * d + cc];
                win[r] = (t >= 0 && t < T) ? v : 0.f;
            }
        }
#pragma unroll
        for (int i = 0; i < DW_TT; ++i) {
            sb += g[i];
#pragma unroll
            for (int jj = 0; jj < KMAX; ++jj) acc[jj] += g[i] * win[i + jj];
        }
    }
    __shared__ float red[3][KMAX + 1][64];
    if (wv > 0) {
#pragma unroll
        for (int jj = 0; jj < KMAX; ++jj) red[wv - 1][jj][lane] = acc[jj];
        red[wv - 1][KMAX][lane] = sb;
    }
    __syncthreads();
    if (wv == 0 && cok) {
        float* row = part + (size_t)blockIdx.x * (KMAX + 1) * d;
#pragma unroll
        for (int jj = 0; jj < KMAX; ++jj)
            row[(size_t)jj * d + c] = (acc[jj] + red[0][jj][lane]) + (red[1][jj][lane] + red[2][jj][lane]);
        row[(size_t)KMAX * d + c] = (sb + red[0][KMAX][lane]) + (red[1][KMAX][lane] + red[2][KMAX][lane]);
    }
}

__global__ __launch_bounds__(256) void dwconv_wgrad_finish_kernel(const float* __restrict__ part, int G, int d, int kmax, int ksz,
                                                                  float* __restrict__ dw, float* __restrict__ db) {
    __shared__ float red[8][32];
    const int o = threadIdx.x & 31, sl = threadIdx.x >> 5;
    const int idx = blockIdx.x * 32 + o, total = (kmax + 1) * d;
    float a0 = 0.f, a1 = 0.f;
    if (idx < total) {
        int g = sl;
        for (; g + 8 < G; g += 16) { a0 += part[(size_t)g * total + idx]; a1 += part[(size_t)(g + 8) * total + idx]; }
        for (; g < G; g += 8) a0 += part[(size_t)g * total + idx];
    }
    red[sl][o] = a0 + a1;
    __syncthreads();
    if (sl != 0 || idx >= total) return;
    const float s = ((red[0][o] + red[1][o]) + (red[2][o] + red[3][o])) + ((red[4][o] + red[5][o]) + (red[6][o] + red[7][o]));
    const int jj = idx / d, c = idx - jj * d;
    if (jj == kmax) {
        if (db) db[c] = s;
    } else {
        const int j = jj - ((kmax - 1) / 2 - (ksz - 1) / 2);
        if (j >= 0 && j < ksz) dw[c * ksz + j] = s;
    }
}

inline int kmax_for(int ksz) { return ksz <= 9 ? 9 : (ksz <= 15 ? 15 : 31); }

inline int wgrad_splits(int B, int T, int d) {
    const int cg = (d + 63) / 64;
    int ns = (768 + B * cg - 1) / (B * cg);
    const int cap = (T + DW_TB - 1) / DW_TB;
    if (ns > cap) ns = cap;
    return ns < 1 ? 1 : ns;
}

inline bool dw_shape_ok(int d, int ksz) { return d > 0 && d <= 4096 && ksz >= 1 && ksz <= 31 && (ksz & 1) == 1; }

}

extern "C" int64_t ia_dwconv_scratch_elems(int B, int T, int d, int ksz) {
    if (B <= 0 || T <= 0 || !dw_shape_ok(d, ksz)) return 0;
    const int64_t fwd = (int64_t)B * ((T + DW_TB - 1) / DW_TB) * 2 * d;
    const int64_t wg = (int64_t)B * wgrad_splits(B, T, d) * (kmax_for(ksz) + 1) * d;
    return fwd > wg ? fwd : wg;
}

extern "C" int ia_glu_dwconv(const void* x2, const int64_t* lens, int B, int T, int d, int ksz, const float* w,
                             const float* bias, float* z, float* bn_sum, float* bn_sumsq, float* scratch,
                             ia_stream_t stream) {
    if (!x2 || !lens || !w || !bias || !z || !bn_sum || !bn_sumsq || !scratch || B <= 0 || T <= 0) return IA_INVALID_VALUE;
    if (!dw_shape_ok(d, ksz)) return IA_UNSUPPORTED;
    hipStream_t st = (hipStream_t)stream;
    const dim3 grid(B * ((T + DW_TB - 1) / DW_TB), (d + 63) / 64), blk(256);
#define IA_DWF(K) hipLaunchKernelGGL((dwconv_fwd_kernel<K, 1>), grid, blk, 0, st, x2, lens, B, T, d, ksz, w, bias, 0, z, scratch, (long long*)nullptr)
    switch (kmax_for(ksz)) {
        case 9: IA_DWF(9); break;
        case 15: IA_DWF(15); break;
        default: IA_DWF(31); break;
    }
#undef IA_DWF
    IA_RETURN_IF_LAUNCH_FAILED();
    ia_partials_finish(scratch, (int)grid.x, 2 * d, d, bn_sum, bn_sumsq, st);
    IA_RETURN_IF_LAUNCH_FAILED();
    return IA_OK;
}

extern "C" int ia_glu_dwconv_fixed(const void* x2, const int64_t* lens, int B, int T, int d, int ksz, const float* w,
                                   const float* bias, float* z, long long* bn_sums_fixed, ia_stream_t stream) {
    if (!x2 || !lens || !w || !bias || !z || !bn_sums_fixed || B <= 0 || T <= 0) return IA_INVALID_VALUE;
    if (!dw_shape_ok(d, ksz)) return IA_UNSUPPORTED;
    hipStream_t st = (hipStream_t)stream;
    const dim3 grid(B * ((T + DW_TB - 1) / DW_TB), (d + 63) / 64), blk(256);
#define IA_DWF(K) hipLaunchKernelGGL((dwconv_fwd_kernel<K, 1>), grid, blk, 0, st, x2, lens, B, T, d, ksz, w, bias, 0, z, (float*)nullptr, bn_sums_fixed)
    switch (kmax_for(ksz)) {
        case 9: IA_DWF(9); break;
        case 15: IA_DWF(15); break;
        default: IA_DWF(31); break;
    }
#undef IA_DWF
    IA_RETURN_IF_LAUNCH_FAILED();
    return IA_OK;
}

extern "C" int ia_dwconv_gated_fixed(const void* g, const int64_t* lens, int B, int T, int d, int ksz, const float* w,
                                     const float* bias, float* z, long long* bn_sums_fixed, ia_stream_t stream) {
    if (!g || !lens || !w || !bias || !z || !bn_sums_fixed || B <= 0 || T <= 0) return IA_INVALID_VALUE;
    if (!dw_shape_ok(d, ksz)) return IA_UNSUPPORTED;
    hipStream_t st = (hipStream_t)stream;
    const dim3 grid(B * ((T + DW_TB - 1) / DW_TB), (d + 63) / 64), blk(256);
#define IA_DWF(K) hipLaunchKernelGGL((dwconv_fwd_kernel<K, 2>), grid, blk, 0, st, g, lens, B, T, d, ksz, w, bias, 0, z, (float*)nullptr, bn_sums_fixed)
    switch (kmax_for(ksz)) {
        case 9: IA_DWF(9); break;
        case 15: IA_DWF(15); break;
        default: IA_DWF(31); break;
    }
#undef IA_DWF
    IA_RETURN_IF_LAUNCH_FAILED();
    return IA_OK;
}

extern "C" int ia_dwconv_time(const float* x, int B, int T, int d, int ksz, const float* w, const float* bias, int flip,
                              float* y, ia_stream_t stream) {
    if (!x || !w || !y || B <= 0 || T <= 0) return IA_INVALID_VALUE;
    if (!dw_shape_ok(d, ksz)) return IA_UNSUPPORTED;
    hipStream_t st = (hipStream_t)stream;
    const dim3 grid(B * ((T + DW_TB - 1) / DW_TB), (d + 63) / 64), blk(256);
#define IA_DWF(K) hipLaunchKernelGGL((dwconv_fwd_kernel<K, 0>), grid, blk, 0, st, (const void*)x, (const int64_t*)nullptr, B, T, d, ksz, w, bias, flip, y, (float*)nullptr, (long long*)nullptr)
    switch (kmax_for(ksz)) {
        case 9: IA_DWF(9); break;
        case 15: IA_DWF(15); break;
        default: IA_DWF(31); break;
    }
#undef IA_DWF
    IA_RETURN_IF_LAUNCH_FAILED();
    return IA_OK;
}

extern "C" int ia_dwconv_time_wgrad(const float* x, const float* dy, int B, int T, int d, int ksz, float* dw, float* db,
                                    float* scratch, ia_stream_t stream) {
    if (!x || !dy || !dw || !scratch || B <= 0 || T <= 0) return IA_INVALID_VALUE;
    if (!dw_shape_ok(d, ksz)) return IA_UNSUPPORTED;
    hipStream_t st = (hipStream_t)stream;
    const int ns = wgrad_splits(B, T, d), kmax = kmax_for(ksz);
    const dim3 grid(B * ns, (d + 63) / 64), blk(256);
#define IA_DWG(K) hipLaunchKernelGGL((dwconv_wgrad_kernel<K, false>), grid, blk, 0, st, x, dy, B, T, d, ns, scratch, (const __bf16*)nullptr, (const int64_t*)nullptr)
    switch (kmax) {
        case 9: IA_DWG(9); break;
        case 15: IA_DWG(15); break;
        default: IA_DWG(31); break;
    }
#undef IA_DWG
    IA_RETURN_IF_LAUNCH_FAILED();
    hipLaunchKernelGGL(dwconv_wgrad_finish_kernel, dim3(((kmax + 1) * d + 31) / 32), dim3(256), 0, st, scratch, (int)grid.x, d,
                       kmax, ksz, dw, db);
    IA_RETURN_IF_LAUNCH_FAILED();
    return IA_OK;
}

extern "C" int ia_dwconv_glu_bwd(const float* dz, const void* c2, const int64_t* lens, int B, int T, int d, int ksz, const float* w,
                                 void* dc2, ia_stream_t stream) {
    if (!dz || !c2 || !lens || !w || !dc2 || B <= 0 || T <= 0) return IA_INVALID_VALUE;
    if (!dw_shape_ok(d, ksz)) return IA_UNSUPPORTED;
    hipStream_t st = (hipStream_t)stream;
    const dim3 grid(B * ((T + DW_TB - 1) / DW_TB), (d + 63) / 64), blk(256);
#define IA_DWF(K) hipLaunchKernelGGL((dwconv_fwd_kernel<K, 3>), grid, blk, 0, st, (const void*)dz, lens, B, T, d, ksz, w, (const float*)nullptr, 1, (float*)nullptr, (float*)nullptr, (long long*)nullptr, (const __bf16*)c2, (__bf16*)dc2)
    switch (kmax_for(ksz)) {
        case 9: IA_DWF(9); break;
        case 15: IA_DWF(15); break;
        default: IA_DWF(31); break;
    }
#undef IA_DWF
    IA_RETURN_IF_LAUNCH_FAILED();
    return IA_OK;
}

extern "C" int ia_dwconv_glu_wgrad(const void* c2, const int64_t* lens, const float* dy, int B, int T, int d, int ksz, float* dw,
                                   float* db, float* scratch, ia_stream_t stream) {
    if (!c2 || !lens || !dy || !dw || !scratch || B <= 0 || T <= 0) return IA_INVALID_VALUE;
    if (!dw_shape_ok(d, ksz)) return IA_UNSUPPORTED;
    hipStream_t st = (hipStream_t)stream;
    const int ns = wgrad_splits(B, T, d), kmax = kmax_for(ksz);
    const dim3 grid(B * ns, (d + 63) / 64), blk(256);
#define IA_DWG(K) hipLaunchKernelGGL((dwconv_wgrad_kernel<K, true>), grid, blk, 0, st, (const float*)nullptr, dy, B, T, d, ns, scratch, (const __bf16*)c2, lens)
    switch (kmax) {
        case 9: IA_DWG(9); break;
        case 15: IA_DWG(15); break;
        default: IA_DWG(31); break;
    }
#undef IA_DWG
    IA_RETURN_IF_LAUNCH_FAILED();
    hipLaunchKernelGGL(dwconv_wgrad_finish_kernel, dim3(((kmax + 1) * d + 31) / 32), dim3(256), 0, st, scratch, (int)grid.x, d,
                       kmax, ksz, dw, db);
    IA_RETURN_IF_LAUNCH_FAILED();
    return IA_OK;
}
```

### indic_cl_asr_amd/csrc/encoder_bwd.hip

```cpp
#include <hip/hip_bf16.h>

#include "dropout_mask.h"
#include <stdlib.h>

#include "ia_common.h"
#include "partials.h"

namespace {

__device__ __forceinline__ float silu_grad(float x) {
    const float s = ia_sigmoid_fast(x);
    return s * (1.f + x * (1.f - s));
}

template <int NV>
__global__ __launch_bounds__(256) void layernorm_bwd_kernel(const float* __restrict__ x, int ldx, const float* __restrict__ dyF,
                                                            const __bf16* __restrict__ dyH, int ldy, int N, int d,
                                                            const float* __restrict__ gamma, float eps,
                                                            const float* __restrict__ dx_in, float* __restrict__ dx_out,
                                                            int lddx, float* __restrict__ part, __bf16* __restrict__ dxh,
                                                            int lddxh, float hscale, unsigned hseed, unsigned hthr, float hks) {
    const int lane = threadIdx.x & 63;
    const int wave0 = blockIdx.x * 4 + (threadIdx.x >> 6), nwaves = gridDim.x * 4;
    const float inv_d = 1.f / (float)d;
    float4 gam[NV], dg[NV], db[NV];
#pragma unroll
    for (int i = 0; i < NV; ++i) {
        const int col = (lane + 64 * i) * 4;
        gam[i] = (col < d) ? *reinterpret_cast<const float4*>(gamma + col) : make_float4(0.f, 0.f, 0.f, 0.f);
        dg[i] = db[i] = make_float4(0.f, 0.f, 0.f, 0.f);
    }
    for (int row = wave0; row < N; row += nwaves) {
        float4 v[NV], g[NV];
        float s = 0.f;
#pragma unroll
        for (int i = 0; i < NV; ++i) {
            const int col = (lane + 64 * i) * 4;
            v[i] = g[i] = make_float4(0.f, 0.f, 0.f, 0.f);
            if (col < d) {
                v[i] = *reinterpret_cast<const float4*>(x + (size_t)row * ldx + col);
                if (dyF) g[i] = *reinterpret_cast<const float4*>(dyF + (size_t)row * ldy + col);
                else {
                    union { uint2 u; __bf16 h[4]; } t;
                    t.u = *reinterpret_cast<const uint2*>(dyH + (size_t)row * ldy + col);
                    g[i] = make_float4((float)t.h[0], (float)t.h[1], (float)t.h[2], (float)t.h[3]);
                }
            }
            s += v[i].x + v[i].y + v[i].z + v[i].w;
        }
        const float mean = ia_wave_sum_dpp(s) * inv_d;
        float q = 0.f;
#pragma unroll
        for (int i = 0; i < NV; ++i)
            if ((lane + 64 * i) * 4 < d) {
                const float a = v[i].x - mean, b = v[i].y - mean, c = v[i].z - mean, e = v[i].w - mean;
                q += a * a + b * b + c * c + e * e;
            }
        const float rstd = rsqrtf(ia_wave_sum_dpp(q) * inv_d + eps);
        float s1 = 0.f, s2 = 0.f;
#pragma unroll
        for (int i = 0; i < NV; ++i)
            if ((lane + 64 * i) * 4 < d) {
                v[i] = make_float4((v[i].x - mean) * rstd, (v[i].y - mean) * rstd, (v[i].z - mean) * rstd, (v[i].w - mean) * rstd);
                dg[i].x += g[i].x * v[i].x; dg[i].y += g[i].y * v[i].y; dg[i].z += g[i].z * v[i].z; dg[i].w += g[i].w * v[i].w;
                db[i].x += g[i].x; db[i].y += g[i].y; db[i].z += g[i].z; db[i].w += g[i].w;
                g[i] = make_float4(g[i].x * gam[i].x, g[i].y * gam[i].y, g[i].z * gam[i].z, g[i].w * gam[i].w);
                s1 += g[i].x + g[i].y + g[i].z + g[i].w;
                s2 += g[i].x * v[i].x + g[i].y * v[i].y + g[i].z * v[i].z + g[i].w * v[i].w;
            }
        const float m1 = ia_wave_sum_dpp(s1) * inv_d, m2 = ia_wave_sum_dpp(s2) * inv_d;
#pragma unroll
        for (int i = 0; i < NV; ++i) {
            const int col = (lane + 64 * i) * 4;
            if (col < d) {
                float4 o = make_float4(rstd * (g[i].x - m1 - v[i].x * m2), rstd * (g[i].y - m1 - v[i].y * m2),
                                       rstd * (g[i].z - m1 - v[i].z * m2), rstd * (g[i].w - m1 - v[i].w * m2));
                if (dx_in) {
                    const float4 p = *reinterpret_cast<const float4*>(dx_in + (size_t)row * lddx + col);
                    o.x += p.x; o.y += p.y; o.z += p.z; o.w += p.w;
                }
                *reinterpret_cast<float4*>(dx_out + (size_t)row * lddx + col) = o;
                if (dxh) {
                    const unsigned m = hthr > 0 ? (ia_keep8(hseed, (unsigned)row, (unsigned)d, (unsigned)(col & ~7), hthr) >> (col & 4)) : 0xFu;
                    union { uint2 u; __bf16 h[4]; } t;
                    t.h[0] = (__bf16)((m & 1u) ? o.x * hscale * hks : 0.f);
                    t.h[1] = (__bf16)((m & 2u) ? o.y * hscale * hks : 0.f);
                    t.h[2] = (__bf16)((m & 4u) ? o.z * hscale * hks : 0.f);
                    t.h[3] = (__bf16)((m & 8u) ? o.w * hscale * hks : 0.f);
                    *reinterpret_cast<uint2*>(dxh + (size_t)row * lddxh + col) = t.u;
                }
            }
        }
    }
    __shared__ float4 red[3][2][NV * 64];
    const int wv = threadIdx.x >> 6;
    if (wv > 0) {
#pragma unroll
        for (int i = 0; i < NV; ++i) { red[wv - 1][0][lane + 64 * i] = dg[i]; red[wv - 1][1][lane + 64 * i] = db[i]; }
    }
    __syncthreads();
    if (wv == 0) {
#pragma unroll
        for (int i = 0; i < NV; ++i) {
            const int col = (lane + 64 * i) * 4;
#pragma unroll
            for (int w = 0; w < 3; ++w) {
                const float4 a = red[w][0][lane + 64 * i], b = red[w][1][lane + 64 * i];
                dg[i].x += a.x; dg[i].y += a.y; dg[i].z += a.z; dg[i].w += a.w;
                db[i].x += b.x; db[i].y += b.y; db[i].z += b.z; db[i].w += b.w;
            }
            if (col < d) {
                *reinterpret_cast<float4*>(part + (size_t)blockIdx.x * 2 * d + col) = dg[i];
                *reinterpret_cast<float4*>(part + (size_t)blockIdx.x * 2 * d + d + col) = db[i];
            }
        }
    }
}

template <int MODE>
__global__ __launch_bounds__(256) void silu_dropout_kernel(const __bf16* __restrict__ a, const __bf16* __restrict__ b, int64_t M,
                                                           int N, unsigned seed, unsigned thr, float keep_scale,
                                                           __bf16* __restrict__ out) {
    const int nv = N / 8;
    const int64_t total = M * nv;
    for (int64_t i = (int64_t)blockIdx.x * 256 + threadIdx.x; i < total; i += (int64_t)gridDim.x * 256) {
        const int64_t gm = i / nv;
        const int gn = (int)(i - gm * nv) * 8;
        union { uint4 u; __bf16 h[8]; } x, y, o;
        x.u = reinterpret_cast<const uint4*>(a)[i];
        if (MODE == 1) y.u = reinterpret_cast<const uint4*>(b)[i];
        const unsigned m = thr > 0 ? ia_keep8(seed, (unsigned)gm, (unsigned)N, (unsigned)gn, thr) : 0xFFu;
#pragma unroll
        for (int j = 0; j < 8; ++j) {
            const float v = (float)x.h[j];
            float r;
            if (MODE == 0) r = ia_silu_fast(v);
            else r = (float)y.h[j] * silu_grad(v);
            o.h[j] = (__bf16)(((m >> j) & 1u) ? r * keep_scale : 0.f);
        }
        reinterpret_cast<uint4*>(out)[i] = o.u;
    }
}

__global__ __launch_bounds__(256) void scale_dropout_bf16_kernel(const float* __restrict__ dy, int64_t M, int N, float alpha,
                                                                 unsigned seed, unsigned thr, float keep_scale,
                                                                 __bf16* __restrict__ out) {
    const int nv = N / 8;
    const int64_t total = M * nv;
    for (int64_t i = (int64_t)blockIdx.x * 256 + threadIdx.x; i < total; i += (int64_t)gridDim.x * 256) {
        const int64_t gm = i / nv;
        const int gn = (int)(i - gm * nv) * 8;
        const float4 p0 = reinterpret_cast<const float4*>(dy)[2 * i], p1 = reinterpret_cast<const float4*>(dy)[2 * i + 1];
        const float v[8] = {p0.x, p0.y, p0.z, p0.w, p1.x, p1.y, p1.z, p1.w};
        const unsigned m = thr > 0 ? ia_keep8(seed, (unsigned)gm, (unsigned)N, (unsigned)gn, thr) : 0xFFu;
        union { uint4 u; __bf16 h[8]; } o;
#pragma unroll
        for (int j = 0; j < 8; ++j) o.h[j] = (__bf16)(((m >> j) & 1u) ? v[j] * alpha * keep_scale : 0.f);
        reinterpret_cast<uint4*>(out)[i] = o.u;
    }
}

__global__ __launch_bounds__(256) void bn_silu_bwd_reduce_kernel(const float* __restrict__ z, const __bf16* __restrict__ dc3,
                                                                 int64_t n_rows, int d, const float* __restrict__ bn_sum,
                                                                 const float* __restrict__ bn_sumsq, const float* __restrict__ gamma,
                                                                 const float* __restrict__ beta, float eps,
                                                                 float* __restrict__ part, int rows_per_block) {
    const int cg = d / 4, nrl = 256 / cg;
    const bool active = (int)threadIdx.x < nrl * cg;
    const int c0 = (active ? (int)threadIdx.x % cg : 0) * 4, rl = active ? (int)threadIdx.x / cg : nrl;
    const float inv_n = 1.f / (float)n_rows;
    float mean[4], rstd[4], gm[4], bt[4], a1[4] = {0, 0, 0, 0}, a2[4] = {0, 0, 0, 0};
#pragma unroll
    for (int j = 0; j < 4; ++j) {
        mean[j] = bn_sum[c0 + j] * inv_n;
        rstd[j] = rsqrtf(fmaxf(bn_sumsq[c0 + j] * inv_n - mean[j] * mean[j], 0.f) + eps);
        gm[j] = gamma[c0 + j]; bt[j] = beta[c0 + j];
    }
    const int64_t r0 = (int64_t)blockIdx.x * rows_per_block;
    const int64_t r1 = (r0 + rows_per_block < n_rows) ? r0 + rows_per_block : n_rows;
    for (int64_t r = r0 + rl; active && r < r1; r += nrl) {
        const float4 zz = *reinterpret_cast<const float4*>(z + r * d + c0);
        union { uint2 u; __bf16 h[4]; } g;
        g.u = *reinterpret_cast<const uint2*>(dc3 + r * d + c0);
        const float zv[4] = {zz.x, zz.y, zz.z, zz.w};
#pragma unroll
        for (int j = 0; j < 4; ++j) {
            const float xh = (zv[j] - mean[j]) * rstd[j];
            const float dyb = (float)g.h[j] * silu_grad(xh * gm[j] + bt[j]);
            a1[j] += dyb; a2[j] += dyb * xh;
        }
    }
    __shared__ float red[2][256][4];
#pragma unroll
    for (int j = 0; j < 4; ++j) { red[0][threadIdx.x][j] = a1[j]; red[1][threadIdx.x][j] = a2[j]; }
    __syncthreads();
    if (rl == 0) {
        for (int k = 1; k < nrl; ++k)
#pragma unroll
            for (int j = 0; j < 4; ++j) { a1[j] += red[0][threadIdx.x + k * cg][j]; a2[j] += red[1][threadIdx.x + k * cg][j]; }
        float* row = part + (size_t)blockIdx.x * 2 * d;
        *reinterpret_cast<float4*>(row + c0) = make_float4(a1[0], a1[1], a1[2], a1[3]);
        *reinterpret_cast<float4*>(row + d + c0) = make_float4(a2[0], a2[1], a2[2], a2[3]);
    }
}
__global__ __launch_bounds__(256) void bn_silu_bwd_apply_kernel(const float* __restrict__ z, const __bf16* __restrict__ dc3,
                                                                int64_t n_rows, int d, const float* __restrict__ bn_sum,
                                                                const float* __restrict__ bn_sumsq, const float* __restrict__ gamma,
                                                                const float* __restrict__ beta, float eps, const float* __restrict__ S1,
                                                                const float* __restrict__ S2, float* __restrict__ dz) {
    const int64_t total4 = n_rows * d / 4;
    const float inv_n = 1.f / (float)n_rows;
    for (int64_t i = (int64_t)blockIdx.x * 256 + threadIdx.x; i < total4; i += (int64_t)gridDim.x * 256) {
        const int c0 = (int)((i * 4) % d);
        const float4 zz = reinterpret_cast<const float4*>(z)[i];
        union { uint2 u; __bf16 h[4]; } g;
        g.u = reinterpret_cast<const uint2*>(dc3)[i];
        const float zv[4] = {zz.x, zz.y, zz.z, zz.w};
        float o[4];
#pragma unroll
        for (int j = 0; j < 4; ++j) {
            const float mean = bn_sum[c0 + j] * inv_n;
            const float rstd = rsqrtf(fmaxf(bn_sumsq[c0 + j] * inv_n - mean * mean, 0.f) + eps);
            const float xh = (zv[j] - mean) * rstd;
            const float dyb = (float)g.h[j] * silu_grad(xh * gamma[c0 + j] + beta[c0 + j]);
            o[j] = gamma[c0 + j] * rstd * (dyb - S1[c0 + j] * inv_n - xh * S2[c0 + j] * inv_n);
        }
        reinterpret_cast<float4*>(dz)[i] = make_float4(o[0], o[1], o[2], o[3]);
    }
}

template <int MODE>
__global__ __launch_bounds__(256) void glu_kernel(const __bf16* __restrict__ c2, const float* __restrict__ dG,
                                                  const int64_t* __restrict__ lens, int B, int T, int d,
                                                  float* __restrict__ G, __bf16* __restrict__ dc2) {
    const int64_t total = (int64_t)B * T * d;
    for (int64_t i = (int64_t)blockIdx.x * 256 + threadIdx.x; i < total; i += (int64_t)gridDim.x * 256) {
        const int c = (int)(i % d);
        const int64_t row = i / d;
        const int t = (int)(row % T), b = (int)(row / T);
        const bool valid = t < (int)lens[b];
        const float a = (float)c2[row * 2 * d + c], g = (float)c2[row * 2 * d + d + c];
        const float sg = ia_sigmoid_fast(g);
        if (MODE == 0) {
            G[i] = valid ? a * sg : 0.f;
        } else {
            const float dg = valid ? dG[i] : 0.f;
            dc2[row * 2 * d + c] = (__bf16)(dg * sg);
            dc2[row * 2 * d + d + c] = (__bf16)(dg * a * sg * (1.f - sg));
        }
    }
}

inline int ew_grid(int64_t items) {
    const int64_t b = (items + 255) / 256;
    return (int)(b < 1 ? 1 : (b > 8192 ? 8192 : b));
}

inline int lnb_blocks(int N) {
    const int b = (N + 7) / 8;
    return b < 1 ? 1 : (b > 1024 ? 1024 : b);
}
}

extern "C" int64_t ia_layernorm_bwd_scratch_elems(int N, int d) { return (N <= 0 || d <= 0) ? 0 : (int64_t)lnb_blocks(N) * 2 * d; }

extern "C" int ia_layernorm_bwd(const float* x, int ldx, const float* dy_f32, const void* dy_bf16, int ldy, int N, int d,
                                const float* gamma, float eps, const float* dx_in, float* dx_out, int lddx, float* dgamma,
                                float* dbeta, float* scratch, ia_stream_t stream) {
    return ia_layernorm_bwd_drop(x, ldx, dy_f32, dy_bf16, ldy, N, d, gamma, eps, dx_in, dx_out, lddx, dgamma, dbeta, 1.f, 0.f, 0,
                                 nullptr, 0, scratch, stream);
}

extern "C" int ia_layernorm_bwd_drop(const float* x, int ldx, const float* dy_f32, const void* dy_bf16, int ldy, int N, int d,
                                     const float* gamma, float eps, const float* dx_in, float* dx_out, int lddx, float* dgamma,
                                     float* dbeta, float alpha, float dropout_p, unsigned seed, void* dx_bf16, int lddxh,
                                     float* scratch, ia_stream_t stream) {
    if (!x || (!dy_f32 && !dy_bf16) || !gamma || !dx_out || ((dgamma == nullptr) != (dbeta == nullptr)) || !scratch || N <= 0 || d <= 0)
        return IA_INVALID_VALUE;
    if (d % 4 != 0 || d > 1024 || ldx % 4 != 0 || ldy % 4 != 0 || lddx % 4 != 0) return IA_UNSUPPORTED;
    if (dx_bf16 && (d % 8 != 0 || lddxh % 4 != 0 || dropout_p < 0.f || dropout_p >= 1.f)) return IA_INVALID_VALUE;
    static const bool split = [] { const char* e = getenv("IA_LN_DROP"); return e && e[0] == '0'; }();
    if (split && dx_bf16) {
        const int st0 = ia_layernorm_bwd_drop(x, ldx, dy_f32, dy_bf16, ldy, N, d, gamma, eps, dx_in, dx_out, lddx, dgamma, dbeta, 1.f, 0.f,
                                              0, nullptr, 0, scratch, stream);
        if (st0 != IA_OK) return st0;
        if (lddx != d || lddxh != d) return IA_UNSUPPORTED;
        return ia_scale_dropout_bf16(dx_out, N, d, alpha, dropout_p, seed, dx_bf16, stream);
    }
    const auto [hthr, hks] = ia_dropout_rule(dropout_p);
    const int G = lnb_blocks(N);
    const dim3 grid(G), blk(256);
    hipStream_t st = (hipStream_t)stream;
    const int nv = (d + 255) / 256;
#define IA_LNB(NV) hipLaunchKernelGGL((layernorm_bwd_kernel<NV>), grid, blk, 0, st, x, ldx, dy_f32, (const __bf16*)dy_bf16, ldy, N, d, gamma, eps, dx_in, dx_out, lddx, scratch, (__bf16*)dx_bf16, lddxh, alpha, seed, hthr, hks)
    switch (nv) {
        case 1: IA_LNB(1); break;
        case 2: IA_LNB(2); break;
        case 3: IA_LNB(3); break;
        default: IA_LNB(4); break;
    }
#undef IA_LNB
    IA_RETURN_IF_LAUNCH_FAILED();
    if (!dgamma) return IA_OK;
    ia_partials_finish(scratch, G, 2 * d, d, dgamma, dbeta, st);
    IA_RETURN_IF_LAUNCH_FAILED();
    return IA_OK;
}

extern "C" int ia_layernorm_bwd_partial_rows(int N) { return N > 0 ? lnb_blocks(N) : 0; }

namespace {
struct FinishJobs { ia_finish_job j[8]; int first_block[9]; int n; };
__global__ __launch_bounds__(1024) void partials_finish_multi_kernel(FinishJobs f) {
    __shared__ float red[16][64];
    int k = 0;
    while (k + 1 < f.n && (int)blockIdx.x >= f.first_block[k + 1]) ++k;
    const ia_finish_job J = f.j[k];
    const int cl = threadIdx.x & 63, rg = threadIdx.x >> 6;
    const int c = ((int)blockIdx.x - f.first_block[k]) * 64 + cl;
    float a0 = 0.f, a1 = 0.f;
    if (c < J.C) {
        int r = rg;
        for (; r + 112 < J.G; r += 128) {
            float v[8];
#pragma unroll
            for (int q = 0; q < 8; ++q) v[q] = J.part[(size_t)(r + 16 * q) * J.C + c];
            a0 += (v[0] + v[2]) + (v[4] + v[6]);
            a1 += (v[1] + v[3]) + (v[5] + v[7]);
        }
        for (; r < J.G; r += 16) a0 += J.part[(size_t)r * J.C + c];
    }
    red[rg][cl] = a0 + a1;
    __syncthreads();
    if (rg == 0 && c < J.C) {
        float s = 0.f;
#pragma unroll
        for (int q = 0; q < 16; ++q) s += red[q][cl];
        if (c < J.C0) J.out0[c] = s; else J.out1[c - J.C0] = s;
    }
}
}

extern "C" int ia_partials_finish_multi(const ia_finish_job* jobs, int count, ia_stream_t stream) {
    if (!jobs || count <= 0 || count > 8) return IA_INVALID_VALUE;
    FinishJobs f;
    f.n = count;
    int blocks = 0;
    for (int i = 0; i < count; ++i) {
        const ia_finish_job& J = jobs[i];
        if (!J.part || !J.out0 || J.G <= 0 || J.C <= 0 || J.C0 < 0 || J.C0 > J.C || (J.C0 < J.C && !J.out1)) return IA_INVALID_VALUE;
        f.j[i] = J;
        f.first_block[i] = blocks;
        blocks += (J.C + 63) / 64;
    }
    f.first_block[count] = blocks;
    hipLaunchKernelGGL(partials_finish_multi_kernel, dim3(blocks), dim3(1024), 0, (hipStream_t)stream, f);
    IA_RETURN_IF_LAUNCH_FAILED();
    return IA_OK;
}

extern "C" int ia_silu_dropout(const void* h_pre, int64_t M, int N, float dropout_p, unsigned seed, void* out, ia_stream_t stream) {
    if (!h_pre || !out || M <= 0 || N <= 0 || N % 8 != 0 || dropout_p < 0.f || dropout_p >= 1.f) return IA_INVALID_VALUE;
    const auto [thr, ks] = ia_dropout_rule(dropout_p);
    hipLaunchKernelGGL((silu_dropout_kernel<0>), dim3(ew_grid(M * (N / 8))), dim3(256), 0, (hipStream_t)stream,
                       (const __bf16*)h_pre, (const __bf16*)nullptr, M, N, seed, thr, ks, (__bf16*)out);
    IA_RETURN_IF_LAUNCH_FAILED();
    return IA_OK;
}

extern "C" int ia_silu_dropout_bwd(const void* h_pre, const void* dh, int64_t M, int N, float dropout_p, unsigned seed, void* out,
                                   ia_stream_t stream) {
    if (!h_pre || !dh || !out || M <= 0 || N <= 0 || N % 8 != 0 || dropout_p < 0.f || dropout_p >= 1.f) return IA_INVALID_VALUE;
    const auto [thr, ks] = ia_dropout_rule(dropout_p);
    hipLaunchKernelGGL((silu_dropout_kernel<1>), dim3(ew_grid(M * (N / 8))), dim3(256), 0, (hipStream_t)stream,
                       (const __bf16*)h_pre, (const __bf16*)dh, M, N, seed, thr, ks, (__bf16*)out);
    IA_RETURN_IF_LAUNCH_FAILED();
    return IA_OK;
}

extern "C" int ia_scale_dropout_bf16(const float* dy, int64_t M, int N, float alpha, float dropout_p, unsigned seed, void* out,
                                     ia_stream_t stream) {
    if (!dy || !out || M <= 0 || N <= 0 || N % 8 != 0 || dropout_p < 0.f || dropout_p >= 1.f) return IA_INVALID_VALUE;
    const auto [thr, ks] = ia_dropout_rule(dropout_p);
    hipLaunchKernelGGL(scale_dropout_bf16_kernel, dim3(ew_grid(M * (N / 8))), dim3(256), 0, (hipStream_t)stream, dy, M, N, alpha,
                       seed, thr, ks, (__bf16*)out);
    IA_RETURN_IF_LAUNCH_FAILED();
    return IA_OK;
}

namespace {
__global__ __launch_bounds__(256) void cast_pad_bf16_kernel(const float* __restrict__ src, int lds, int64_t M, int N,
                                                            __bf16* __restrict__ dst, int ldd) {
    const int vpr = ldd / 8;
    const int64_t total = M * vpr;
    for (int64_t i = (int64_t)blockIdx.x * 256 + threadIdx.x; i < total; i += (int64_t)gridDim.x * 256) {
        const int64_t m = i / vpr;
        const int n0 = (int)(i - m * vpr) * 8;
        const float* s = src + m * lds + n0;
        union { uint4 u; __bf16 h[8]; } o;
#pragma unroll
        for (int j = 0; j < 8; ++j) o.h[j] = (__bf16)((n0 + j < N) ? s[j] : 0.f);
        *reinterpret_cast<uint4*>(dst + m * ldd + n0) = o.u;
    }
}
}

extern "C" int ia_cast_pad_bf16(const float* src, int lds, int64_t M, int N, void* dst, int ldd, ia_stream_t stream) {
    if (!src || !dst || M <= 0 || N <= 0 || lds < N || ldd < N || ldd % 8 != 0 || !ia_is_aligned(dst, 16)) return IA_INVALID_VALUE;
    hipLaunchKernelGGL(cast_pad_bf16_kernel, dim3(ew_grid(M * (ldd / 8))), dim3(256), 0, (hipStream_t)stream, src, lds, M, N,
                       (__bf16*)dst, ldd);
    IA_RETURN_IF_LAUNCH_FAILED();
    return IA_OK;
}

namespace {
inline int bnb_rows_per_block(int64_t n_rows) {
    int64_t rpb = (n_rows + 1023) / 1024;
    return (int)(rpb < 32 ? 32 : rpb);
}
}

extern "C" int64_t ia_bn_silu_bwd_scratch_elems(int64_t n_rows, int d) {
    if (n_rows <= 0 || d <= 0) return 0;
    const int rpb = bnb_rows_per_block(n_rows);
    return ((n_rows + rpb - 1) / rpb) * 2 * (int64_t)d;
}

extern "C" int ia_bn_silu_bwd(const float* z, const void* dc3, int64_t n_rows, int d, const float* bn_sum, const float* bn_sumsq,
                              const float* gamma, const float* beta, float eps, float* S1, float* S2, float* dz,
                              float* scratch, ia_stream_t stream) {
    if (!z || !dc3 || !bn_sum || !bn_sumsq || !gamma || !beta || !S1 || !S2 || !dz || !scratch || n_rows <= 1 || d <= 0)
        return IA_INVALID_VALUE;
    if (d % 4 != 0 || d > 1024) return IA_UNSUPPORTED;
    hipStream_t st = (hipStream_t)stream;
    const int rpb = bnb_rows_per_block(n_rows);
    const int G = (int)((n_rows + rpb - 1) / rpb);
    hipLaunchKernelGGL(bn_silu_bwd_reduce_kernel, dim3((unsigned)G), dim3(256), 0, st, z, (const __bf16*)dc3, n_rows, d, bn_sum,
                       bn_sumsq, gamma, beta, eps, scratch, rpb);
    IA_RETURN_IF_LAUNCH_FAILED();
    ia_partials_finish(scratch, G, 2 * d, d, S1, S2, st);
    IA_RETURN_IF_LAUNCH_FAILED();
    hipLaunchKernelGGL(bn_silu_bwd_apply_kernel, dim3(ew_grid(n_rows * d / 4)), dim3(256), 0, st, z, (const __bf16*)dc3, n_rows, d,
                       bn_sum, bn_sumsq, gamma, beta, eps, S1, S2, dz);
    IA_RETURN_IF_LAUNCH_FAILED();
    return IA_OK;
}

extern "C" int ia_bn_silu_bwd_reduce(const float* z, const void* dc3, int64_t n_rows, int d, const float* bn_sum,
                                     const float* bn_sumsq, const float* gamma, const float* beta, float eps, float* S1, float* S2,
                                     float* scratch, ia_stream_t stream) {
    if (!z || !dc3 || !bn_sum || !bn_sumsq || !gamma || !beta || !S1 || !S2 || !scratch || n_rows <= 1 || d <= 0)
        return IA_INVALID_VALUE;
    if (d % 4 != 0 || d > 1024) return IA_UNSUPPORTED;
    hipStream_t st = (hipStream_t)stream;
    const int rpb = bnb_rows_per_block(n_rows);
    const int G = (int)((n_rows + rpb - 1) / rpb);
    hipLaunchKernelGGL(bn_silu_bwd_reduce_kernel, dim3((unsigned)G), dim3(256), 0, st, z, (const __bf16*)dc3, n_rows, d, bn_sum,
                       bn_sumsq, gamma, beta, eps, scratch, rpb);
    IA_RETURN_IF_LAUNCH_FAILED();
    ia_partials_finish(scratch, G, 2 * d, d, S1, S2, st);
    IA_RETURN_IF_LAUNCH_FAILED();
    return IA_OK;
}

extern "C" int ia_bn_silu_bwd_apply(const float* z, const void* dc3, int64_t n_rows, int d, const float* bn_sum,
                                    const float* bn_sumsq, const float* gamma, const float* beta, float eps, const float* S1,
                                    const float* S2, float* dz, ia_stream_t stream) {
    if (!z || !dc3 || !bn_sum || !bn_sumsq || !gamma || !beta || !S1 || !S2 || !dz || n_rows <= 1 || d <= 0) return IA_INVALID_VALUE;
    if (d % 4 != 0) return IA_UNSUPPORTED;
    hipLaunchKernelGGL(bn_silu_bwd_apply_kernel, dim3(ew_grid(n_rows * d / 4)), dim3(256), 0, (hipStream_t)stream, z,
                       (const __bf16*)dc3, n_rows, d, bn_sum, bn_sumsq, gamma, beta, eps, S1, S2, dz);
    IA_RETURN_IF_LAUNCH_FAILED();
    return IA_OK;
}

extern "C" int ia_glu_mask(const void* c2, const int64_t* lens, int B, int T, int d, float* G, ia_stream_t stream) {
    if (!c2 || !lens || !G || B <= 0 || T <= 0 || d <= 0) return IA_INVALID_VALUE;
    hipLaunchKernelGGL((glu_kernel<0>), dim3(ew_grid((int64_t)B * T * d)), dim3(256), 0, (hipStream_t)stream, (const __bf16*)c2,
                       (const float*)nullptr, lens, B, T, d, G, (__bf16*)nullptr);
    IA_RETURN_IF_LAUNCH_FAILED();
    return IA_OK;
}

extern "C" int ia_glu_bwd(const void* c2, const float* dG, const int64_t* lens, int B, int T, int d, void* dc2, ia_stream_t stream) {
    if (!c2 || !dG || !lens || !dc2 || B <= 0 || T <= 0 || d <= 0) return IA_INVALID_VALUE;
    hipLaunchKernelGGL((glu_kernel<1>), dim3(ew_grid((int64_t)B * T * d)), dim3(256), 0, (hipStream_t)stream, (const __bf16*)c2, dG,
                       lens, B, T, d, (float*)nullptr, (__bf16*)dc2);
    IA_RETURN_IF_LAUNCH_FAILED();
    return IA_OK;
}
```

### indic_cl_asr_amd/csrc/gemm_tn.hip

```cpp
#include <hip/hip_bf16.h>

#include "ia_common.h"
#include "lds_transpose.h"
#include "partials.h"

namespace {

typedef __bf16 bf8 __attribute__((ext_vector_type(8)));
typedef __bf16 bf4 __attribute__((ext_vector_type(4)));
typedef float f4 __attribute__((ext_vector_type(4)));

constexpr int TN_BN = 128;
constexpr int TN_BK = 128;
constexpr int TN_MS = 64;
constexpr int TN_ROWB = 256;
constexpr int TN_TILE = TN_MS * TN_ROWB;


__device__ __forceinline__ bool tn_map(int local, int tiles, int S, int* tile, int* split) {
    const int xcd = local & 7, slot = local >> 3;
    if (S >= 8) {
        *split = (slot / tiles) * 8 + xcd; *tile = slot % tiles;
        return *split < S;
    }
    const int G = 8 / S;
    *split = xcd % S; *tile = slot * G + xcd / S;
    return *tile < tiles;
}
inline int tn_round_splits(int s) { return s >= 8 ? s / 8 * 8 : (s >= 4 ? 4 : (s >= 2 ? 2 : 1)); }
inline int tn_plan_splits(int M, int wanted, int* rps_out) {
    int S = tn_round_splits(wanted < 1 ? 1 : wanted);
    for (;;) {
        int rps = (M + S - 1) / S;
        rps = (rps + TN_MS - 1) / TN_MS * TN_MS;
        const int Seff = (M + rps - 1) / rps;
        if (Seff >= 8 || Seff == tn_round_splits(Seff)) { *rps_out = rps; return Seff; }
        S = tn_round_splits(Seff);
    }
}
inline int tn_wgs(int tiles, int S) { return S >= 8 ? 8 * ((S + 7) / 8) * tiles : 8 * ((tiles + 8 / S - 1) / (8 / S)); }

__device__ __forceinline__ void tn_tile_body(const __bf16* __restrict__ dY, int ldy, const __bf16* __restrict__ X, int ldx, int M,
                                             int n, int k, int rows_per_split, float* __restrict__ part,
                                             float* __restrict__ part_b, size_t row_stride, int tile, int split,
                                             unsigned char* smem) {
    unsigned char* sY = smem;
    unsigned char* sX = smem + TN_TILE;
    const unsigned ldsY = (unsigned)(size_t)((__attribute__((address_space(3))) unsigned char*)sY);
    const unsigned ldsX = ldsY + TN_TILE;
    const int tid = threadIdx.x, lane = tid & 63, wave = tid >> 6;
    const int c = lane & 15, q4 = lane >> 4;
    const int wn = wave >> 1, wk = wave & 1;
    const int ntk = (k + TN_BK - 1) / TN_BK;
    const int n0 = (tile / ntk) * TN_BN, k0 = (tile % ntk) * TN_BK;
    const int m_beg = split * rows_per_split;
    int m_end = m_beg + rows_per_split; m_end = m_end < M ? m_end : M;
    const bool do_bias = part_b != nullptr && k0 == 0 && wk == 0;

    f4 acc[4][4], accb[4];
#pragma unroll
    for (int i = 0; i < 4; ++i) {
        accb[i] = (f4){0.f, 0.f, 0.f, 0.f};
#pragma unroll
        for (int j = 0; j < 4; ++j) acc[i][j] = (f4){0.f, 0.f, 0.f, 0.f};
    }
    bf8 ones;
#pragma unroll
    for (int j = 0; j < 8; ++j) ones[j] = (__bf16)1.f;

    auto multiply_stage = [&](unsigned lY, unsigned lX) {
#pragma unroll
        for (int ks = 0; ks < TN_MS / 32; ++ks) {
            bf4 alo[4], ahi[4], blo[4], bhi[4];
#pragma unroll
            for (int i = 0; i < 4; ++i) {
                unsigned a0, a1;
                trl_frag_addr<false>(lY, TN_ROWB, ks * 32 + q4 * 8, wn * 64 + i * 16, lane, &a0, &a1);
                alo[i] = trl_read<bf4>(a0); ahi[i] = trl_read<bf4>(a1);
                trl_frag_addr<false>(lX, TN_ROWB, ks * 32 + q4 * 8, wk * 64 + i * 16, lane, &a0, &a1);
                blo[i] = trl_read<bf4>(a0); bhi[i] = trl_read<bf4>(a1);
            }
            asm volatile("s_waitcnt lgkmcnt(0)"
                         : "+v"(alo[0]), "+v"(alo[1]), "+v"(alo[2]), "+v"(alo[3]), "+v"(ahi[0]), "+v"(ahi[1]), "+v"(ahi[2]),
                           "+v"(ahi[3]), "+v"(blo[0]), "+v"(blo[1]), "+v"(blo[2]), "+v"(blo[3]), "+v"(bhi[0]), "+v"(bhi[1]),
                           "+v"(bhi[2]), "+v"(bhi[3])
                         :
                         : "memory");
            bf8 af[4], bfr[4];
#pragma unroll
            for (int i = 0; i < 4; ++i) { af[i] = trl_join(alo[i], ahi[i]); bfr[i] = trl_join(blo[i], bhi[i]); }
#pragma unroll
            for (int i = 0; i < 4; ++i) {
#pragma unroll
                for (int j = 0; j < 4; ++j) acc[i][j] = __builtin_amdgcn_mfma_f32_16x16x32_bf16(af[i], bfr[j], acc[i][j], 0, 0, 0);
                if (do_bias) accb[i] = __builtin_amdgcn_mfma_f32_16x16x32_bf16(af[i], ones, accb[i], 0, 0, 0);
            }
        }
    };

    const bool dma_path = n0 + TN_BN <= n && k0 + TN_BK <= k && (m_end - m_beg) % TN_MS == 0 && m_end > m_beg;
    if (dma_path) {
        const unsigned char* gy = reinterpret_cast<const unsigned char*>(dY + (size_t)m_beg * ldy + n0);
        const unsigned char* gx = reinterpret_cast<const unsigned char*>(X + (size_t)m_beg * ldx + k0);
        const int wv = __builtin_amdgcn_readfirstlane(wave);
        unsigned oy[4], ox[4];
#pragma unroll
        for (int i = 0; i < 4; ++i) {
            const int row = 4 * (wv * 4 + i) + (lane >> 4);
            const unsigned ch = (unsigned)((lane & 15) ^ (((lane >> 4) << 2) | i));
            oy[i] = (unsigned)row * (unsigned)(ldy * 2) + ch * 16u;
            ox[i] = (unsigned)row * (unsigned)(ldx * 2) + ch * 16u;
        }
        auto issue = [&](int st, int buf) {
            const unsigned char* py = gy + (size_t)st * TN_MS * ldy * 2;
            const unsigned char* px = gx + (size_t)st * TN_MS * ldx * 2;
            unsigned char* dy_ = smem + buf * 2 * TN_TILE + wv * 4096;
#pragma unroll
            for (int i = 0; i < 4; ++i)
                __builtin_amdgcn_global_load_lds((const __attribute__((address_space(1))) void*)(py + oy[i]),
                                                 (__attribute__((address_space(3))) void*)(dy_ + i * 1024), 16, 0, 0);
#pragma unroll
            for (int i = 0; i < 4; ++i)
                __builtin_amdgcn_global_load_lds((const __attribute__((address_space(1))) void*)(px + ox[i]),
                                                 (__attribute__((address_space(3))) void*)(dy_ + TN_TILE + i * 1024), 16, 0, 0);
        };
        const int nst = (m_end - m_beg) / TN_MS;
        issue(0, 0);
        for (int st = 0; st < nst; ++st) {
            asm volatile("s_waitcnt vmcnt(0)" ::: "memory");
            __builtin_amdgcn_s_barrier();
            if (st + 1 < nst) issue(st + 1, (st + 1) & 1);
            const unsigned base = ldsY + (unsigned)((st & 1) * 2 * TN_TILE);
            multiply_stage(base, base + TN_TILE);
        }
    } else {
    uint4 ry[4], rx[4];
#define TN_LOAD(m0_)                                                                                               \
    do {                                                                                                           \
        _Pragma("unroll") for (int i = 0; i < 4; ++i) {                                                            \
            const int idx_ = tid + 256 * i, row_ = idx_ >> 4, ch_ = idx_ & 15;                                     \
            const int m_ = (m0_) + row_;                                                                           \
            const bool okm_ = m_ < m_end;                                                                          \
            const int cy_ = n0 + ch_ * 8, cx_ = k0 + ch_ * 8;                                                      \
            ry[i] = (okm_ && cy_ < n) ? *reinterpret_cast<const uint4*>(dY + (size_t)m_ * ldy + cy_) : make_uint4(0, 0, 0, 0); \
            rx[i] = (okm_ && cx_ < k) ? *reinterpret_cast<const uint4*>(X + (size_t)m_ * ldx + cx_) : make_uint4(0, 0, 0, 0);  \
        }                                                                                                          \
    } while (0)
#define TN_STORE()                                                                                                 \
    do {                                                                                                           \
        _Pragma("unroll") for (int i = 0; i < 4; ++i) {                                                            \
            const int idx_ = tid + 256 * i, row_ = idx_ >> 4, ch_ = idx_ & 15;                                     \
            *reinterpret_cast<uint4*>(sY + trl_off<false>(TN_ROWB, row_, ch_)) = ry[i];                                             \
            *reinterpret_cast<uint4*>(sX + trl_off<false>(TN_ROWB, row_, ch_)) = rx[i];                                             \
        }                                                                                                          \
    } while (0)

    TN_LOAD(m_beg);
    for (int m0 = m_beg; m0 < m_end; m0 += TN_MS) {
        __syncthreads();
        TN_STORE();
        __syncthreads();
        if (m0 + TN_MS < m_end) TN_LOAD(m0 + TN_MS);
        multiply_stage(ldsY, ldsX);
    }
    }
#undef TN_LOAD
#undef TN_STORE
    float* prow = part + (size_t)split * row_stride;
#pragma unroll
    for (int i = 0; i < 4; ++i)
#pragma unroll
        for (int r = 0; r < 4; ++r) {
            const int gn = n0 + wn * 64 + i * 16 + q4 * 4 + r;
            if (gn < n) {
#pragma unroll
                for (int j = 0; j < 4; ++j) {
                    const int gk = k0 + wk * 64 + j * 16 + c;
                    if (gk < k) prow[(size_t)gn * k + gk] = acc[i][j][r];
                }
                if (do_bias && c == 0) part_b[(size_t)split * row_stride + gn] = accb[i][r];
            }
        }
}

__global__ __launch_bounds__(256, 2) void gemm_tn_kernel(const __bf16* __restrict__ dY, int ldy, const __bf16* __restrict__ X,
                                                         int ldx, int M, int n, int k, int rows_per_split,
                                                         float* __restrict__ part, float* __restrict__ part_b,
                                                         size_t row_stride) {
    __shared__ __attribute__((aligned(16))) unsigned char smem[4 * TN_TILE];
    const int tiles = ((n + TN_BN - 1) / TN_BN) * ((k + TN_BK - 1) / TN_BK);
    const int S = (M + rows_per_split - 1) / rows_per_split;
    int tile, split;
    if (!tn_map((int)blockIdx.x, tiles, S, &tile, &split)) return;
    tn_tile_body(dY, ldy, X, ldx, M, n, k, rows_per_split, part, part_b, row_stride, tile, split, smem);
}

constexpr int TN_MAX_GROUP = 12;
struct TnProblem {
    const __bf16* dY; const __bf16* X; float* part; float* part_b; float* dW; float* db;
    size_t row_stride; int ldy, ldx, M, n, k, rps, S, tiles, wg_begin; int64_t out_begin;
};
struct TnGroup { TnProblem p[TN_MAX_GROUP]; int count; };

__global__ __launch_bounds__(256, 2) void gemm_tn_grouped_kernel(TnGroup g) {
    __shared__ __attribute__((aligned(16))) unsigned char smem[4 * TN_TILE];
    int pi = 0;
#pragma unroll
    for (int i = 1; i < TN_MAX_GROUP; ++i)
        if (i < g.count && (int)blockIdx.x >= g.p[i].wg_begin) pi = i;
    pi = __builtin_amdgcn_readfirstlane(pi);
    const TnProblem& P = g.p[pi];
    int tile, split;
    if (!tn_map((int)blockIdx.x - P.wg_begin, P.tiles, P.S, &tile, &split)) return;
    tn_tile_body(P.dY, P.ldy, P.X, P.ldx, P.M, P.n, P.k, P.rps, P.part, P.part_b, P.row_stride, tile, split, smem);
}

__global__ __launch_bounds__(256) void gemm_tn_grouped_finish_kernel(TnGroup g, int64_t total4) {
    for (int64_t i = (int64_t)blockIdx.x * 256 + threadIdx.x; i < total4; i += (int64_t)gridDim.x * 256) {
        const int64_t e = i * 4;
        int pi = 0;
#pragma unroll
        for (int j = 1; j < TN_MAX_GROUP; ++j)
            if (j < g.count && e >= g.p[j].out_begin) pi = j;
        const TnProblem& P = g.p[pi];
        const int64_t off = e - P.out_begin;
        const int64_t nk = (int64_t)P.n * P.k;
        if (off >= nk && !P.db) continue;
        float4 a = make_float4(0.f, 0.f, 0.f, 0.f);
        const float* src = P.part + off;
        for (int s_ = 0; s_ < P.S; ++s_) {
            const float4 x = *reinterpret_cast<const float4*>(src + (size_t)s_ * P.row_stride);
            a.x += x.x; a.y += x.y; a.z += x.z; a.w += x.w;
        }
        float* dst = off < nk ? P.dW + off : P.db + (off - nk);
        *reinterpret_cast<float4*>(dst) = a;
    }
}

inline int tn_splits(int M, int n, int k) {
    const int tiles = ((n + TN_BN - 1) / TN_BN) * ((k + TN_BK - 1) / TN_BK);
    int s = (320 + tiles - 1) / tiles;
    const int cap = (M + TN_MS - 1) / TN_MS;
    s = s < 1 ? 1 : (s > cap ? cap : s);
    return s;
}
}

extern "C" int64_t ia_gemm_tn_scratch_elems(int M, int n, int k) {
    if (M <= 0 || n <= 0 || k <= 0) return 0;
    return (int64_t)tn_splits(M, n, k) * ((int64_t)n * k + n);
}

extern "C" int ia_gemm_tn_bf16(const void* dY, int ldy, const void* X, int ldx, int M, int n, int k, float* dW, float* db,
                               float* scratch, ia_stream_t stream) {
    if (!dY || !X || !dW || !scratch || M <= 0 || n <= 0 || k <= 0) return IA_INVALID_VALUE;
    if (n % 8 != 0 || k % 8 != 0 || ldy % 8 != 0 || ldx % 8 != 0 || !ia_is_aligned(dY, 16) || !ia_is_aligned(X, 16)) return IA_UNSUPPORTED;
    int rps;
    const int Seff = tn_plan_splits(M, tn_splits(M, n, k), &rps);
    const size_t row_stride = (size_t)n * k + n;
    float* part = scratch;
    float* part_b = db ? scratch + (size_t)n * k : nullptr;
    hipStream_t st = (hipStream_t)stream;
    const dim3 grid(tn_wgs(((n + TN_BN - 1) / TN_BN) * ((k + TN_BK - 1) / TN_BK), Seff)), blk(256);
    hipLaunchKernelGGL(gemm_tn_kernel, grid, blk, 0, st, (const __bf16*)dY, ldy, (const __bf16*)X, ldx, M, n, k, rps, part, part_b,
                       row_stride);
    IA_RETURN_IF_LAUNCH_FAILED();
    if (db == dW + (size_t)n * k) {
        ia_partials_finish_wide(part, Seff, (int64_t)row_stride, dW, st);
    } else {
        ia_partials_finish_wide_strided(part, Seff, (int64_t)n * k, (int64_t)row_stride, dW, st);
        if (db) {
            IA_RETURN_IF_LAUNCH_FAILED();
            ia_partials_finish_wide_strided(part_b, Seff, (int64_t)n, (int64_t)row_stride, db, st);
        }
    }
    IA_RETURN_IF_LAUNCH_FAILED();
    return IA_OK;
}

namespace {
inline int tn_group_plan(const ia_tn_problem* pr, int count, TnGroup* g, int64_t* scratch_elems, int64_t* out_elems, int* blocks) {
    if (!pr || count <= 0 || count > TN_MAX_GROUP) return IA_INVALID_VALUE;
    int tiles_total = 0;
    for (int i = 0; i < count; ++i) {
        const ia_tn_problem& q = pr[i];
        if (q.M <= 0 || q.n <= 0 || q.k <= 0) return IA_INVALID_VALUE;
        if (q.n % 8 != 0 || q.k % 8 != 0 || q.ldy % 8 != 0 || q.ldx % 8 != 0) return IA_UNSUPPORTED;
        tiles_total += ((q.n + TN_BN - 1) / TN_BN) * ((q.k + TN_BK - 1) / TN_BK);
    }
    int S0 = 512 / tiles_total;
    S0 = S0 < 1 ? 1 : S0;
    int64_t so = 0, oo = 0;
    int wg = 0;
    g->count = count;
    for (int i = 0; i < count; ++i) {
        const ia_tn_problem& q = pr[i];
        TnProblem& P = g->p[i];
        const int cap = (q.M + TN_MS - 1) / TN_MS;
        int rps;
        const int S = tn_plan_splits(q.M, S0 > cap ? cap : S0, &rps);
        P.dY = (const __bf16*)q.dY; P.X = (const __bf16*)q.X; P.ldy = q.ldy; P.ldx = q.ldx; P.M = q.M; P.n = q.n; P.k = q.k;
        P.rps = rps; P.S = S; P.tiles = ((q.n + TN_BN - 1) / TN_BN) * ((q.k + TN_BK - 1) / TN_BK);
        P.row_stride = (size_t)q.n * q.k + q.n;
        P.part = nullptr; P.part_b = nullptr;
        P.dW = q.dW; P.db = q.db;
        P.wg_begin = wg; wg += tn_wgs(P.tiles, S);
        P.out_begin = oo; oo += (int64_t)P.row_stride;
        P.part = reinterpret_cast<float*>(so * sizeof(float));
        so += (int64_t)S * (int64_t)P.row_stride;
        so = (so + 3) / 4 * 4;
    }
    *scratch_elems = so; *out_elems = oo; *blocks = wg;
    return IA_OK;
}
}

extern "C" int64_t ia_gemm_tn_grouped_scratch_elems(const ia_tn_problem* problems, int count) {
    TnGroup g; int64_t so = 0, oo = 0; int blocks = 0;
    if (tn_group_plan(problems, count, &g, &so, &oo, &blocks) != IA_OK) return 0;
    return so;
}

extern "C" int ia_gemm_tn_bf16_grouped(const ia_tn_problem* problems, int count, float* scratch, ia_stream_t stream) {
    if (!scratch) return IA_INVALID_VALUE;
    TnGroup g; int64_t so = 0, oo = 0; int blocks = 0;
    const int rc = tn_group_plan(problems, count, &g, &so, &oo, &blocks);
    if (rc != IA_OK) return rc;
    for (int i = 0; i < count; ++i) {
        TnProblem& P = g.p[i];
        if (!P.dY || !P.X || !P.dW || !ia_is_aligned(P.dY, 16) || !ia_is_aligned(P.X, 16) || !ia_is_aligned(P.dW, 16) ||
            (P.db && !ia_is_aligned(P.db, 16)))
            return IA_INVALID_VALUE;
        P.part = scratch + reinterpret_cast<size_t>(P.part) / sizeof(float);
        P.part_b = P.db ? P.part + (size_t)P.n * P.k : nullptr;
    }
    hipStream_t st = (hipStream_t)stream;
    hipLaunchKernelGGL(gemm_tn_grouped_kernel, dim3(blocks), dim3(256), 0, st, g);
    IA_RETURN_IF_LAUNCH_FAILED();
    const int64_t total4 = oo / 4;
    const int64_t fb = (total4 + 255) / 256;
    hipLaunchKernelGGL(gemm_tn_grouped_finish_kernel, dim3((unsigned)(fb < 2048 ? fb : 2048)), dim3(256), 0, st, g, total4);
    IA_RETURN_IF_LAUNCH_FAILED();
    return IA_OK;
}
```

### indic_cl_asr_amd/csrc/partials.h

```cpp
#pragma once
#include <hip/hip_runtime.h>

namespace {
__global__ __launch_bounds__(1024) void ia_partials_finish_kernel(const float* __restrict__ part, int G, int C, int C0,
                                                                  float* __restrict__ out0, float* __restrict__ out1) {
    __shared__ float red[16][64];
    const int cl = threadIdx.x & 63, rg = threadIdx.x >> 6;
    const int c = blockIdx.x * 64 + cl;
    float a0 = 0.f, a1 = 0.f;
    if (c < C) {
        int r = rg;
        for (; r + 112 < G; r += 128) {
            float v[8];
#pragma unroll
            for (int k = 0; k < 8; ++k) v[k] = part[(size_t)(r + 16 * k) * C + c];
            a0 += (v[0] + v[2]) + (v[4] + v[6]);
            a1 += (v[1] + v[3]) + (v[5] + v[7]);
        }
        for (; r < G; r += 16) a0 += part[(size_t)r * C + c];
    }
    red[rg][cl] = a0 + a1;
    __syncthreads();
    if (rg == 0 && c < C) {
        float s = 0.f;
#pragma unroll
        for (int k = 0; k < 16; ++k) s += red[k][cl];
        if (c < C0) out0[c] = s; else out1[c - C0] = s;
    }
}

__global__ __launch_bounds__(256) void ia_partials_finish_wide_kernel(const float* __restrict__ part, int G, int64_t C4,
                                                                      int64_t S4, float* __restrict__ out) {
    for (int64_t i = (int64_t)blockIdx.x * 256 + threadIdx.x; i < C4; i += (int64_t)gridDim.x * 256) {
        const float4* p = reinterpret_cast<const float4*>(part) + i;
        float4 a = make_float4(0.f, 0.f, 0.f, 0.f), b = a;
        int g = 0;
        for (; g + 1 < G; g += 2) {
            const float4 x = p[(int64_t)g * S4], y = p[(int64_t)(g + 1) * S4];
            a.x += x.x; a.y += x.y; a.z += x.z; a.w += x.w;
            b.x += y.x; b.y += y.y; b.z += y.z; b.w += y.w;
        }
        if (g < G) { const float4 x = p[(int64_t)g * S4]; a.x += x.x; a.y += x.y; a.z += x.z; a.w += x.w; }
        reinterpret_cast<float4*>(out)[i] = make_float4(a.x + b.x, a.y + b.y, a.z + b.z, a.w + b.w);
    }
}

inline void ia_partials_finish_wide_strided(const float* part, int G, int64_t C, int64_t stride, float* out, hipStream_t st) {
    const int64_t c4 = C / 4, blocks = (c4 + 255) / 256;
    hipLaunchKernelGGL(ia_partials_finish_wide_kernel, dim3((unsigned)(blocks < 4096 ? blocks : 4096)), dim3(256), 0, st, part, G,
                       c4, stride / 4, out);
}
inline void ia_partials_finish_wide(const float* part, int G, int64_t C, float* out, hipStream_t st) {
    ia_partials_finish_wide_strided(part, G, C, C, out, st);
}

inline void ia_partials_finish(const float* part, int G, int C, int C0, float* out0, float* out1, hipStream_t st) {
    hipLaunchKernelGGL(ia_partials_finish_kernel, dim3((C + 63) / 64), dim3(1024), 0, st, part, G, C, C0, out0, out1);
}
}
```

Before: 3789 utterances/s.

## Fold split-K partial reductions into downstream consumer kernels to cut launches

Split-K partial reductions are no longer finished by separate kernels. The grouped TN weight-gradient GEMM, the depthwise-conv wgrad and the layernorm partials now publish descriptors of their partial buffers. Those partials are summed inside one combined kernel that also does the gradient accumulation adds. In attention backward, the dpos GEMM partials are summed directly in the dpos pack kernel. This removes several finish launches and one round trip of the reduced fp32 outputs through memory per layer. In exchange, the combined kernel carries a per-element lookup of the add table and more complex branching, and the path can be turned off with an environment variable.

```diff
diff --git a/indic_cl_asr_amd/csrc/attention_flash_bwd.hip b/indic_cl_asr_amd/csrc/attention_flash_bwd.hip
--- a/indic_cl_asr_amd/csrc/attention_flash_bwd.hip
+++ b/indic_cl_asr_amd/csrc/attention_flash_bwd.hip
@@ -514,8 +514,10 @@
     }
 }
 
+template <bool PARTIALS>
 __global__ __launch_bounds__(256) void fb_dpos_pack_kernel(const float* __restrict__ dpos, int H, int Rs, int pad0, int R, int dk,
-                                                           int rows, __bf16* __restrict__ out) {
+                                                           int rows, __bf16* __restrict__ out, const float* __restrict__ part,
+                                                           int64_t head_step, int S, int64_t stride) {
     const int d = H * dk, q = dk / 4;
     const int64_t total = (int64_t)rows * H * q;
     for (int64_t i = (int64_t)blockIdx.x * 256 + threadIdx.x; i < total; i += (int64_t)gridDim.x * 256) {
@@ -525,7 +527,9 @@
         union { uint2 u; __bf16 e[4]; } o;
         o.u = make_uint2(0, 0);
         if (r < R) {
-            const float4 v = *reinterpret_cast<const float4*>(dpos + (size_t)h * ((size_t)Rs * 64 + Rs) + (size_t)(pad0 + r) * 64 + e4 * 4);
+            const size_t at = (size_t)(pad0 + r) * 64 + e4 * 4;
+            const float4 v = PARTIALS ? ia_chain_sum4(part + (size_t)h * head_step + at, S, (size_t)stride)
+                                      : *reinterpret_cast<const float4*>(dpos + (size_t)h * ((size_t)Rs * 64 + Rs) + at);
             o.e[0] = (__bf16)v.x; o.e[1] = (__bf16)v.y; o.e[2] = (__bf16)v.z; o.e[3] = (__bf16)v.w;
         }
         *reinterpret_cast<uint2*>(out + (size_t)r * d + h * dk + e4 * 4) = o.u;
@@ -619,6 +623,28 @@
     ia_partials_finish(a.part, B * nt, 2 * H * dk, H * dk, dbias_u, dbias_v, st);
     IA_RETURN_IF_LAUNCH_FAILED();
     float* dpos = ws + w.dpos;
+    const int64_t items = (int64_t)pl_rows * H * (dk / 4);
+    const int64_t blocks = (items + 255) / 256;
+    const dim3 pgrid((unsigned)(blocks < 4096 ? blocks : 4096));
+    if (H <= 8 && ia_inlaunch_finish()) {
+        ia_tn_problem pr[8];
+        ia_partial_src src[16];
+        int nsrc = 0;
+        for (int h = 0; h < H; ++h)
+            pr[h] = ia_tn_problem{(const __bf16*)dBand + (size_t)h * B * T * rs, (const __bf16*)QvHM + (size_t)h * B * T * 64,
+                                  dpos + (size_t)h * ((size_t)rs * 64 + rs), nullptr, rs, 64, B * T, rs, 64};
+        const int rc = ia_gemm_tn_grouped_partials(pr, H, ws + w.tn, src, &nsrc, stream);
+        if (rc != IA_OK) return rc;
+        const int64_t step = H > 1 ? src[1].part - src[0].part : 0;
+        bool regular = nsrc == H;
+        for (int h = 0; regular && h < H; ++h)
+            regular = src[h].G == src[0].G && src[h].stride == src[0].stride && src[h].part == src[0].part + h * step;
+        if (!regular) return IA_UNSUPPORTED;
+        hipLaunchKernelGGL(fb_dpos_pack_kernel<true>, pgrid, dim3(256), 0, st, (const float*)dpos, H, rs, p0, 2 * T - 1, dk, pl_rows,
+                           (__bf16*)dpl, src[0].part, step, src[0].G, src[0].stride);
+        IA_RETURN_IF_LAUNCH_FAILED();
+        return IA_OK;
+    }
     for (int h0 = 0; h0 < H; h0 += 8) {
         ia_tn_problem pr[8];
         const int nh = H - h0 < 8 ? H - h0 : 8;
@@ -631,10 +657,8 @@
         const int rc = ia_gemm_tn_bf16_grouped(pr, nh, ws + w.tn, stream);
         if (rc != IA_OK) return rc;
     }
-    const int64_t items = (int64_t)pl_rows * H * (dk / 4);
-    const int64_t blocks = (items + 255) / 256;
-    hipLaunchKernelGGL(fb_dpos_pack_kernel, dim3((unsigned)(blocks < 4096 ? blocks : 4096)), dim3(256), 0, st, (const float*)dpos, H, rs,
-                       p0, 2 * T - 1, dk, pl_rows, (__bf16*)dpl);
+    hipLaunchKernelGGL(fb_dpos_pack_kernel<false>, pgrid, dim3(256), 0, st, (const float*)dpos, H, rs, p0, 2 * T - 1, dk, pl_rows,
+                       (__bf16*)dpl, (const float*)nullptr, (int64_t)0, 0, (int64_t)0);
     IA_RETURN_IF_LAUNCH_FAILED();
     return IA_OK;
 }
diff --git a/indic_cl_asr_amd/csrc/block_train.hip b/indic_cl_asr_amd/csrc/block_train.hip
--- a/indic_cl_asr_amd/csrc/block_train.hip
+++ b/indic_cl_asr_amd/csrc/block_train.hip
@@ -6,6 +6,7 @@
 #include <cstdlib>
 
 #include "ia_common.h"
+#include "partials.h"
 
 namespace {
 
@@ -94,22 +95,132 @@
 }
 
 struct AddRow { float* dst; const float* src; int64_t n; };
+__device__ __forceinline__ void add_range(float* __restrict__ dst, const float* __restrict__ src, int64_t n, int bx, int nbx) {
+    const int64_t n4 = ((reinterpret_cast<uintptr_t>(dst) | reinterpret_cast<uintptr_t>(src)) & 15) ? 0 : (n >> 2);
+    for (int64_t i = (int64_t)bx * 256 + threadIdx.x; i < n4; i += (int64_t)nbx * 256) {
+        float4 a = reinterpret_cast<float4*>(dst)[i];
+        const float4 b = reinterpret_cast<const float4*>(src)[i];
+        a.x += b.x; a.y += b.y; a.z += b.z; a.w += b.w;
+        reinterpret_cast<float4*>(dst)[i] = a;
+    }
+    for (int64_t i = (n4 << 2) + (int64_t)bx * 256 + threadIdx.x; i < n; i += (int64_t)nbx * 256) dst[i] += src[i];
+}
 __global__ __launch_bounds__(256) void multi_add_kernel(const AddRow* __restrict__ table, int rows) {
     for (int k = blockIdx.y; k < rows; k += gridDim.y) {
         const AddRow r = table[k];
-        const int64_t n4 = ((reinterpret_cast<uintptr_t>(r.dst) | reinterpret_cast<uintptr_t>(r.src)) & 15) ? 0 : (r.n >> 2);
-        for (int64_t i = (int64_t)blockIdx.x * 256 + threadIdx.x; i < n4; i += (int64_t)gridDim.x * 256) {
-            float4 a = reinterpret_cast<float4*>(r.dst)[i];
-            const float4 b = reinterpret_cast<const float4*>(r.src)[i];
-            a.x += b.x; a.y += b.y; a.z += b.z; a.w += b.w;
-            reinterpret_cast<float4*>(r.dst)[i] = a;
-        }
-        for (int64_t i = (n4 << 2) + (int64_t)blockIdx.x * 256 + threadIdx.x; i < r.n; i += (int64_t)gridDim.x * 256) r.dst[i] += r.src[i];
+        add_range(r.dst, r.src, r.n, blockIdx.x, gridDim.x);
+    }
+}
+
+constexpr int MAX_SRC = 32, MAX_HIT = 64, PLAIN_X = 8, PLAIN_ROWS = 64;
+struct PartialSrcs { ia_partial_src s[MAX_SRC]; int first_block[MAX_SRC + 1]; int n; };
+
+inline int src_blocks(const ia_partial_src& S) {
+    switch (S.kind) {
+        case IA_SUM_CHAIN: return (S.len + 1023) / 1024;
+        case IA_SUM_COLS: return (S.len + 15) / 16;
+        case IA_SUM_SLICES: return (S.len + 31) / 32;
+        default: return (S.d * S.ksz + 31) / 32;
+    }
+}
+
+__device__ __forceinline__ const AddRow* find_row(const AddRow* list, int cnt, const float* p) {
+    for (int j = 0; j < cnt; ++j)
+        if (p >= list[j].src && p < list[j].src + list[j].n) return &list[j];
+    return nullptr;
+}
+__device__ __forceinline__ void put1(const AddRow* list, int cnt, float* o, float v) {
+    const AddRow* r = find_row(list, cnt, o);
+    if (r) { float* q = r->dst + (o - r->src); *q += v; } else *o = v;
+}
+
+__global__ __launch_bounds__(256) void multi_add_combine_kernel(const AddRow* __restrict__ table, int rows, PartialSrcs ps) {
+    __shared__ float red[16 * 17];
+    __shared__ AddRow hit[MAX_HIT];
+    __shared__ int nhit;
+    const int bid = blockIdx.x, tid = threadIdx.x;
+    if (bid >= ps.first_block[ps.n]) {
+        const int pb = bid - ps.first_block[ps.n];
+        for (int k = pb / PLAIN_X; k < rows; k += PLAIN_ROWS) {
+            const AddRow r = table[k];
+            bool claimed = false;
+            for (int j = 0; j < ps.n; ++j) claimed = claimed || (r.src >= ps.s[j].out && r.src < ps.s[j].out + ps.s[j].len);
+            if (!claimed) add_range(r.dst, r.src, r.n, pb % PLAIN_X, PLAIN_X);
+        }
+        return;
+    }
+    int si = 0;
+    for (int j = 1; j < ps.n; ++j)
+        if (bid >= ps.first_block[j]) si = j;
+    si = __builtin_amdgcn_readfirstlane(si);
+    const ia_partial_src& S = ps.s[si];
+    const int chunk = bid - ps.first_block[si];
+    AddRow mine = AddRow{nullptr, nullptr, 0};
+    if (tid < rows) mine = table[tid];
+    if (tid == 0) nhit = 0;
+
+    float4 v4 = make_float4(0.f, 0.f, 0.f, 0.f);
+    float v = 0.f;
+    int64_t e = -1;
+    bool vec = false;
+    if (S.kind == IA_SUM_CHAIN) {
+        e = (int64_t)chunk * 1024 + tid * 4;
+        vec = (reinterpret_cast<uintptr_t>(S.part) & 15) == 0 && (S.stride & 3) == 0 && e + 4 <= S.len;
+        if (vec) {
+            v4 = ia_chain_sum4(S.part + e, S.G, (size_t)S.stride);
+        } else if (e < S.len) {
+            float t[4] = {0.f, 0.f, 0.f, 0.f};
+            for (int i = 0; i < 4 && e + i < S.len; ++i) t[i] = ia_chain_sum1(S.part + e + i, S.G, (size_t)S.stride);
+            v4 = make_float4(t[0], t[1], t[2], t[3]);
+        }
+    } else if (S.kind == IA_SUM_COLS) {
+        const int cl = tid & 15, rg = tid >> 4;
+        const int64_t i = (int64_t)chunk * 16 + cl;
+        red[rg * 17 + cl] = i < S.len ? ia_colsum_rowgroup(S.part, S.G, (int)S.stride, (int)(S.col0 + i), rg) : 0.f;
+        if (rg == 0 && i < S.len) e = i;
+    } else {
+        const bool taps = S.kind == IA_SUM_TAPS;
+        const int o = tid & 31, sl = tid >> 5;
+        const int64_t q = (int64_t)chunk * 32 + o, ncol = taps ? (int64_t)S.d * S.ksz : S.len;
+        red[sl * 33 + o] = q < ncol ? ia_slicesum_slice(S.part, S.G, S.stride, S.col0 + q, sl) : 0.f;
+        if (sl == 0 && q < ncol) {
+            if (taps) { const int64_t j = q / S.d, c = q - j * S.d; e = c * S.ksz + j; } else e = q;
+        }
+    }
+    __syncthreads();
+    for (int j = tid; j < rows; j += 256) {
+        const AddRow r = j == tid ? mine : table[j];
+        if (r.src < S.out + S.len && r.src + r.n > S.out) {
+            const int h = atomicAdd(&nhit, 1);
+            if (h < MAX_HIT) hit[h] = r;
+        }
+    }
+    if (S.kind == IA_SUM_COLS) { if (e >= 0) v = ia_colsum_16(red + (tid & 15), 17); }
+    else if (S.kind != IA_SUM_CHAIN) { if (e >= 0) v = ia_slicesum_8(red + (tid & 31), 33); }
+    __syncthreads();
+    const bool in_lds = nhit <= MAX_HIT;
+    const AddRow* list = in_lds ? hit : table;
+    const int cnt = in_lds ? nhit : rows;
+    if (S.kind != IA_SUM_CHAIN) {
+        if (e >= 0) put1(list, cnt, S.out + e, v);
+        return;
+    }
+    if (e >= S.len) return;
+    float* o = S.out + e;
+    const AddRow* r = vec ? find_row(list, cnt, o) : nullptr;
+    if (r && o + 4 <= r->src + r->n && (reinterpret_cast<uintptr_t>(r->dst + (o - r->src)) & 15) == 0) {
+        float4* q = reinterpret_cast<float4*>(r->dst + (o - r->src));
+        float4 a = *q;
+        a.x += v4.x; a.y += v4.y; a.z += v4.z; a.w += v4.w;
+        *q = a;
+    } else {
+        const float t[4] = {v4.x, v4.y, v4.z, v4.w};
+        for (int i = 0; i < 4 && e + i < S.len; ++i) put1(list, cnt, o + i, t[i]);
     }
 }
 
 struct BwdWs {
-    size_t dxa, dxb, dB, dB1, dB2, dB3, dh, dhp, dy, dc3, dz, dG, dc2, dctx, wt, scr, total;
+    size_t dxa, dxb, dB, dB1, dB2, dB3, dh, dhp, dy, dc3, dz, dG, dc2, dctx, wt, scr, dwp, total;
 };
 
 size_t max3(size_t a, size_t b, size_t c) { return a > b ? (a > c ? a : c) : (b > c ? b : c); }
@@ -158,6 +269,7 @@
         scr = scr > (size_t)ia_gemm_tn_grouped_scratch_elems(gall, 9) ? scr : (size_t)ia_gemm_tn_grouped_scratch_elems(gall, 9);
     }
     w.scr = o;  o = up256(o + scr * 4);
+    w.dwp = o;  o = up256(o + (size_t)ia_dwconv_scratch_elems(B, T, d, ksz) * 4);
     w.total = o;
     return w;
 }
@@ -211,7 +323,7 @@
     }
     return c.ok ? &c : nullptr;
 }
-struct PendingGroup { ia_tn_problem grp[8]; int n = 0; const void* ws = nullptr; };
+struct PendingGroup { ia_tn_problem grp[8]; int n = 0; const void* ws = nullptr; ia_partial_src dw[2]; int ndw = 0; };
 PendingGroup* pending_group() {
     static PendingGroup pg[16];
     int dev = 0;
@@ -350,9 +462,14 @@
     IA_TRY(ia_dwconv_glu_bwd(dz, S.c2, lens, B, T, d, ksz, L.dw_w, dc2, stream));
     SideCtx* side = phase == 0 ? side_ctx() : nullptr;
     hipStream_t main = (hipStream_t)stream;
+    const bool carry = !side && phase == 0 && merged_wgrads() && pending_group();
+    if (carry) pending_group()->ndw = 0;
     if (side) {
         IA_TRY(stream_after(main, side->s, side->ev[0]));
         IA_TRY(ia_dwconv_glu_wgrad(S.c2, lens, dz, B, T, d, ksz, G.dw_w, G.dw_b, scr, (ia_stream_t)side->s));
+    } else if (carry && ia_inlaunch_finish()) {
+        PendingGroup* pg = pending_group();
+        IA_TRY(ia_dwconv_glu_wgrad_partials(S.c2, lens, dz, B, T, d, ksz, G.dw_w, G.dw_b, (float*)(ws + w.dwp), pg->dw, &pg->ndw, stream));
     } else {
         IA_TRY(ia_dwconv_glu_wgrad(S.c2, lens, dz, B, T, d, ksz, G.dw_w, G.dw_b, scr, stream));
     }
@@ -365,7 +482,7 @@
         IA_TRY(flush_group(grp, ngrp, scr, (ia_stream_t)side->s));
         if (hipEventRecord(side->ev[2], side->s) != hipSuccess) return IA_LAUNCH_FAILED;
         side->a_pending = true;
-    } else if (phase == 0 && merged_wgrads() && pending_group()) {
+    } else if (carry) {
         PendingGroup* pg = pending_group();
         for (int i = 0; i < ngrp; ++i) pg->grp[i] = grp[i];
         pg->n = ngrp; pg->ws = workspace;
@@ -398,9 +515,12 @@
     const float p = L.p_drop, pff = L.p_ff;
     ia_tn_problem grp[12];
     int ngrp = 0;
+    ia_partial_src dwsrc[2];
+    int ndw = 0;
     if (carried) {
         for (int i = 0; i < pg->n; ++i) grp[ngrp++] = pg->grp[i];
-        pg->n = 0;
+        for (int i = 0; i < pg->ndw; ++i) dwsrc[ndw++] = pg->dw[i];
+        pg->n = 0; pg->ndw = 0;
     }
     char* wtb = (char*)wt + ((size_t)2 * d * d_ff + (size_t)4 * d * d) * 2;
     void *wt_qkv = wtb, *wt_ff1b = wtb + (size_t)3 * d * d * 2, *wt_ff1a = wtb + ((size_t)3 * d * d + (size_t)d * d_ff) * 2;
@@ -437,11 +557,23 @@
         IA_TRY(linear_bwd_deferred(dhp, S.y1, L.w_ff1a, N, d_ff, d, dy, G.w_ff1a, G.b_ff1a, wt_ff1a, grp, &ngrp, stream));
     }
     IA_TRY(ia_layernorm_bwd(x0, d, nullptr, dy, d, N, d, L.ln_ff1_g, L.ln_eps, dxb, dx0, d, nullptr, nullptr, lnp + 4 * lnp_set, stream));
+    const bool combine = !side && add_table && n_add > 0 && tn_grouping_enabled() && 2 * ngrp + 12 <= MAX_SRC && ia_inlaunch_finish();
+    PartialSrcs ps;
+    ps.n = 0;
     if (side) {
         IA_TRY(stream_after(main, side->s, side->ev[5]));
         stream = (ia_stream_t)side->s;
+    } else if (combine) {
+        IA_TRY(ia_gemm_tn_grouped_partials(grp, ngrp, scr, ps.s, &ps.n, stream));
     } else {
         IA_TRY(flush_group(grp, ngrp, scr, stream));
+    }
+    if (ndw > 0) {
+        if (combine) {
+            for (int i = 0; i < ndw; ++i) ps.s[ps.n++] = dwsrc[i];
+        } else {
+            IA_TRY(ia_dwconv_wgrad_finish(dwsrc[0].part, dwsrc[0].G, d, ksz, G.dw_w, ndw > 1 ? G.dw_b : nullptr, stream));
+        }
     }
     {
         const int rows = ia_layernorm_bwd_partial_rows(N);
@@ -450,9 +582,23 @@
                                        {lnp + 2 * lnp_set, rows, 2 * d, d, G.ln_conv_g, G.ln_conv_b},
                                        {lnp + 3 * lnp_set, rows, 2 * d, d, G.ln_att_g, G.ln_att_b},
                                        {lnp + 4 * lnp_set, rows, 2 * d, d, G.ln_ff1_g, G.ln_ff1_b}};
-        IA_TRY(ia_partials_finish_multi(jobs, 5, stream));
-    }
-    if (add_table && n_add > 0) {
+        if (combine) {
+            for (int i = 0; i < 5; ++i) {
+                ps.s[ps.n++] = ia_partial_src{jobs[i].out0, jobs[i].part, 2 * d, d, rows, IA_SUM_COLS, 0, 0, 0};
+                ps.s[ps.n++] = ia_partial_src{jobs[i].out1, jobs[i].part, 2 * d, d, rows, IA_SUM_COLS, d, 0, 0};
+            }
+        } else {
+            IA_TRY(ia_partials_finish_multi(jobs, 5, stream));
+        }
+    }
+    if (combine) {
+        int blocks = 0;
+        for (int i = 0; i < ps.n; ++i) { ps.first_block[i] = blocks; blocks += src_blocks(ps.s[i]); }
+        ps.first_block[ps.n] = blocks;
+        blocks += PLAIN_X * (n_add < PLAIN_ROWS ? n_add : PLAIN_ROWS);
+        hipLaunchKernelGGL(multi_add_combine_kernel, dim3(blocks), dim3(256), 0, (hipStream_t)stream, (const AddRow*)add_table, n_add, ps);
+        IA_RETURN_IF_LAUNCH_FAILED();
+    } else if (add_table && n_add > 0) {
         hipLaunchKernelGGL(multi_add_kernel, dim3(64, n_add < 64 ? n_add : 64), dim3(256), 0, (hipStream_t)stream,
                            (const AddRow*)add_table, n_add);
         IA_RETURN_IF_LAUNCH_FAILED();
diff --git a/indic_cl_asr_amd/csrc/dwconv.hip b/indic_cl_asr_amd/csrc/dwconv.hip
--- a/indic_cl_asr_amd/csrc/dwconv.hip
+++ b/indic_cl_asr_amd/csrc/dwconv.hip
@@ -166,16 +166,10 @@
     __shared__ float red[8][32];
     const int o = threadIdx.x & 31, sl = threadIdx.x >> 5;
     const int idx = blockIdx.x * 32 + o, total = (kmax + 1) * d;
-    float a0 = 0.f, a1 = 0.f;
-    if (idx < total) {
-        int g = sl;
-        for (; g + 8 < G; g += 16) { a0 += part[(size_t)g * total + idx]; a1 += part[(size_t)(g + 8) * total + idx]; }
-        for (; g < G; g += 8) a0 += part[(size_t)g * total + idx];
-    }
-    red[sl][o] = a0 + a1;
+    red[sl][o] = idx < total ? ia_slicesum_slice(part, G, total, idx, sl) : 0.f;
     __syncthreads();
     if (sl != 0 || idx >= total) return;
-    const float s = ((red[0][o] + red[1][o]) + (red[2][o] + red[3][o])) + ((red[4][o] + red[5][o]) + (red[6][o] + red[7][o]));
+    const float s = ia_slicesum_8(&red[0][o], 32);
     const int jj = idx / d, c = idx - jj * d;
     if (jj == kmax) {
         if (db) db[c] = s;
@@ -315,8 +309,8 @@
     return IA_OK;
 }
 
-extern "C" int ia_dwconv_glu_wgrad(const void* c2, const int64_t* lens, const float* dy, int B, int T, int d, int ksz, float* dw,
-                                   float* db, float* scratch, ia_stream_t stream) {
+int ia_dwconv_glu_wgrad_partials(const void* c2, const int64_t* lens, const float* dy, int B, int T, int d, int ksz, float* dw,
+                                 float* db, float* scratch, ia_partial_src* src, int* nsrc, void* stream) {
     if (!c2 || !lens || !dy || !dw || !scratch || B <= 0 || T <= 0) return IA_INVALID_VALUE;
     if (!dw_shape_ok(d, ksz)) return IA_UNSUPPORTED;
     hipStream_t st = (hipStream_t)stream;
@@ -330,8 +324,27 @@
     }
 #undef IA_DWG
     IA_RETURN_IF_LAUNCH_FAILED();
-    hipLaunchKernelGGL(dwconv_wgrad_finish_kernel, dim3(((kmax + 1) * d + 31) / 32), dim3(256), 0, st, scratch, (int)grid.x, d,
+    if (src && nsrc) {
+        const int64_t total = (int64_t)(kmax + 1) * d;
+        int m = 0;
+        src[m++] = ia_partial_src{dw, scratch, total, d * ksz, (int)grid.x, IA_SUM_TAPS, ((kmax - 1) / 2 - (ksz - 1) / 2) * d, d, ksz};
+        if (db) src[m++] = ia_partial_src{db, scratch, total, d, (int)grid.x, IA_SUM_SLICES, kmax * d, d, ksz};
+        *nsrc = m;
+    }
+    return IA_OK;
+}
+
+int ia_dwconv_wgrad_finish(const float* part, int G, int d, int ksz, float* dw, float* db, void* stream) {
+    const int kmax = kmax_for(ksz);
+    hipLaunchKernelGGL(dwconv_wgrad_finish_kernel, dim3(((kmax + 1) * d + 31) / 32), dim3(256), 0, (hipStream_t)stream, part, G, d,
                        kmax, ksz, dw, db);
     IA_RETURN_IF_LAUNCH_FAILED();
     return IA_OK;
 }
+
+extern "C" int ia_dwconv_glu_wgrad(const void* c2, const int64_t* lens, const float* dy, int B, int T, int d, int ksz, float* dw,
+                                   float* db, float* scratch, ia_stream_t stream) {
+    const int rc = ia_dwconv_glu_wgrad_partials(c2, lens, dy, B, T, d, ksz, dw, db, scratch, nullptr, nullptr, stream);
+    if (rc != IA_OK) return rc;
+    return ia_dwconv_wgrad_finish(scratch, B * wgrad_splits(B, T, d), d, ksz, dw, db, stream);
+}
diff --git a/indic_cl_asr_amd/csrc/encoder_bwd.hip b/indic_cl_asr_amd/csrc/encoder_bwd.hip
--- a/indic_cl_asr_amd/csrc/encoder_bwd.hip
+++ b/indic_cl_asr_amd/csrc/encoder_bwd.hip
@@ -318,24 +318,10 @@
     const ia_finish_job J = f.j[k];
     const int cl = threadIdx.x & 63, rg = threadIdx.x >> 6;
     const int c = ((int)blockIdx.x - f.first_block[k]) * 64 + cl;
-    float a0 = 0.f, a1 = 0.f;
-    if (c < J.C) {
-        int r = rg;
-        for (; r + 112 < J.G; r += 128) {
-            float v[8];
-#pragma unroll
-            for (int q = 0; q < 8; ++q) v[q] = J.part[(size_t)(r + 16 * q) * J.C + c];
-            a0 += (v[0] + v[2]) + (v[4] + v[6]);
-            a1 += (v[1] + v[3]) + (v[5] + v[7]);
-        }
-        for (; r < J.G; r += 16) a0 += J.part[(size_t)r * J.C + c];
-    }
-    red[rg][cl] = a0 + a1;
+    red[rg][cl] = c < J.C ? ia_colsum_rowgroup(J.part, J.G, J.C, c, rg) : 0.f;
     __syncthreads();
     if (rg == 0 && c < J.C) {
-        float s = 0.f;
-#pragma unroll
-        for (int q = 0; q < 16; ++q) s += red[q][cl];
+        const float s = ia_colsum_16(&red[0][cl], 64);
         if (c < J.C0) J.out0[c] = s; else J.out1[c - J.C0] = s;
     }
 }
diff --git a/indic_cl_asr_amd/csrc/gemm_tn.hip b/indic_cl_asr_amd/csrc/gemm_tn.hip
--- a/indic_cl_asr_amd/csrc/gemm_tn.hip
+++ b/indic_cl_asr_amd/csrc/gemm_tn.hip
@@ -226,12 +226,7 @@
         const int64_t off = e - P.out_begin;
         const int64_t nk = (int64_t)P.n * P.k;
         if (off >= nk && !P.db) continue;
-        float4 a = make_float4(0.f, 0.f, 0.f, 0.f);
-        const float* src = P.part + off;
-        for (int s_ = 0; s_ < P.S; ++s_) {
-            const float4 x = *reinterpret_cast<const float4*>(src + (size_t)s_ * P.row_stride);
-            a.x += x.x; a.y += x.y; a.z += x.z; a.w += x.w;
-        }
+        const float4 a = ia_chain_sum4(P.part + off, P.S, P.row_stride);
         float* dst = off < nk ? P.dW + off : P.db + (off - nk);
         *reinterpret_cast<float4*>(dst) = a;
     }
@@ -321,10 +316,12 @@
     return so;
 }
 
-extern "C" int ia_gemm_tn_bf16_grouped(const ia_tn_problem* problems, int count, float* scratch, ia_stream_t stream) {
+namespace {
+int tn_group_launch(const ia_tn_problem* problems, int count, float* scratch, TnGroup* gp, int64_t* out_elems, hipStream_t st) {
     if (!scratch) return IA_INVALID_VALUE;
-    TnGroup g; int64_t so = 0, oo = 0; int blocks = 0;
-    const int rc = tn_group_plan(problems, count, &g, &so, &oo, &blocks);
+    TnGroup& g = *gp;
+    int64_t so = 0; int blocks = 0;
+    const int rc = tn_group_plan(problems, count, &g, &so, out_elems, &blocks);
     if (rc != IA_OK) return rc;
     for (int i = 0; i < count; ++i) {
         TnProblem& P = g.p[i];
@@ -334,9 +331,33 @@
         P.part = scratch + reinterpret_cast<size_t>(P.part) / sizeof(float);
         P.part_b = P.db ? P.part + (size_t)P.n * P.k : nullptr;
     }
-    hipStream_t st = (hipStream_t)stream;
     hipLaunchKernelGGL(gemm_tn_grouped_kernel, dim3(blocks), dim3(256), 0, st, g);
     IA_RETURN_IF_LAUNCH_FAILED();
+    return IA_OK;
+}
+}
+
+int ia_gemm_tn_grouped_partials(const ia_tn_problem* problems, int count, float* scratch, ia_partial_src* src, int* nsrc,
+                                void* stream) {
+    if (!src || !nsrc) return IA_INVALID_VALUE;
+    TnGroup g; int64_t oo = 0;
+    const int rc = tn_group_launch(problems, count, scratch, &g, &oo, (hipStream_t)stream);
+    if (rc != IA_OK) return rc;
+    int m = 0;
+    for (int i = 0; i < count; ++i) {
+        const TnProblem& P = g.p[i];
+        src[m++] = ia_partial_src{P.dW, P.part, (int64_t)P.row_stride, P.n * P.k, P.S, IA_SUM_CHAIN, 0, 0, 0};
+        if (P.db) src[m++] = ia_partial_src{P.db, P.part_b, (int64_t)P.row_stride, P.n, P.S, IA_SUM_CHAIN, 0, 0, 0};
+    }
+    *nsrc = m;
+    return IA_OK;
+}
+
+extern "C" int ia_gemm_tn_bf16_grouped(const ia_tn_problem* problems, int count, float* scratch, ia_stream_t stream) {
+    TnGroup g; int64_t oo = 0;
+    hipStream_t st = (hipStream_t)stream;
+    const int rc = tn_group_launch(problems, count, scratch, &g, &oo, st);
+    if (rc != IA_OK) return rc;
     const int64_t total4 = oo / 4;
     const int64_t fb = (total4 + 255) / 256;
     hipLaunchKernelGGL(gemm_tn_grouped_finish_kernel, dim3((unsigned)(fb < 2048 ? fb : 2048)), dim3(256), 0, st, g, total4);
diff --git a/indic_cl_asr_amd/csrc/partials.h b/indic_cl_asr_amd/csrc/partials.h
--- a/indic_cl_asr_amd/csrc/partials.h
+++ b/indic_cl_asr_amd/csrc/partials.h
@@ -1,5 +1,82 @@
 #pragma once
 #include <hip/hip_runtime.h>
+
+#include <cstdint>
+#include <cstdlib>
+
+__device__ __forceinline__ float ia_colsum_rowgroup(const float* __restrict__ part, int G, int C, int c, int rg) {
+    float a0 = 0.f, a1 = 0.f;
+    int r = rg;
+    for (; r + 112 < G; r += 128) {
+        float v[8];
+#pragma unroll
+        for (int k = 0; k < 8; ++k) v[k] = part[(size_t)(r + 16 * k) * C + c];
+        a0 += (v[0] + v[2]) + (v[4] + v[6]);
+        a1 += (v[1] + v[3]) + (v[5] + v[7]);
+    }
+    for (; r < G; r += 16) a0 += part[(size_t)r * C + c];
+    return a0 + a1;
+}
+__device__ __forceinline__ float ia_colsum_16(const float* red, int stride) {
+    float s = 0.f;
+#pragma unroll
+    for (int k = 0; k < 16; ++k) s += red[k * stride];
+    return s;
+}
+__device__ __forceinline__ float4 ia_wide_sum4(const float4* __restrict__ p, int G, int64_t S4) {
+    float4 a = make_float4(0.f, 0.f, 0.f, 0.f), b = a;
+    int g = 0;
+    for (; g + 1 < G; g += 2) {
+        const float4 x = p[(int64_t)g * S4], y = p[(int64_t)(g + 1) * S4];
+        a.x += x.x; a.y += x.y; a.z += x.z; a.w += x.w;
+        b.x += y.x; b.y += y.y; b.z += y.z; b.w += y.w;
+    }
+    if (g < G) { const float4 x = p[(int64_t)g * S4]; a.x += x.x; a.y += x.y; a.z += x.z; a.w += x.w; }
+    return make_float4(a.x + b.x, a.y + b.y, a.z + b.z, a.w + b.w);
+}
+__device__ __forceinline__ float4 ia_chain_sum4(const float* __restrict__ src, int S, size_t stride) {
+    float4 a = make_float4(0.f, 0.f, 0.f, 0.f);
+    for (int s_ = 0; s_ < S; ++s_) {
+        const float4 x = *reinterpret_cast<const float4*>(src + (size_t)s_ * stride);
+        a.x += x.x; a.y += x.y; a.z += x.z; a.w += x.w;
+    }
+    return a;
+}
+__device__ __forceinline__ float ia_chain_sum1(const float* __restrict__ src, int S, size_t stride) {
+    float a = 0.f;
+    for (int s_ = 0; s_ < S; ++s_) a += src[(size_t)s_ * stride];
+    return a;
+}
+
+__device__ __forceinline__ float ia_slicesum_slice(const float* __restrict__ part, int G, int64_t total, int64_t idx, int sl) {
+    float a0 = 0.f, a1 = 0.f;
+    int g = sl;
+    for (; g + 8 < G; g += 16) { a0 += part[(size_t)g * total + idx]; a1 += part[(size_t)(g + 8) * total + idx]; }
+    for (; g < G; g += 8) a0 += part[(size_t)g * total + idx];
+    return a0 + a1;
+}
+__device__ __forceinline__ float ia_slicesum_8(const float* red, int stride) {
+    return ((red[0] + red[stride]) + (red[2 * stride] + red[3 * stride])) +
+           ((red[4 * stride] + red[5 * stride]) + (red[6 * stride] + red[7 * stride]));
+}
+
+enum { IA_SUM_CHAIN = 0, IA_SUM_COLS = 1, IA_SUM_SLICES = 2, IA_SUM_TAPS = 3 };
+struct ia_partial_src {
+    float* out;
+    const float* part;
+    int64_t stride;
+    int len, G, kind;
+    int col0, d, ksz;
+};
+inline bool ia_inlaunch_finish() {
+    const char* e = getenv("IA_INLAUNCH_FINISH");
+    return !(e && e[0] == '0');
+}
+int ia_gemm_tn_grouped_partials(const struct ia_tn_problem* problems, int count, float* scratch, ia_partial_src* src, int* nsrc,
+                                void* stream);
+int ia_dwconv_glu_wgrad_partials(const void* c2, const int64_t* lens, const float* dy, int B, int T, int d, int ksz, float* dw,
+                                 float* db, float* scratch, ia_partial_src* src, int* nsrc, void* stream);
+int ia_dwconv_wgrad_finish(const float* part, int G, int d, int ksz, float* dw, float* db, void* stream);
 
 namespace {
 __global__ __launch_bounds__(1024) void ia_partials_finish_kernel(const float* __restrict__ part, int G, int C, int C0,
@@ -7,42 +84,18 @@
     __shared__ float red[16][64];
     const int cl = threadIdx.x & 63, rg = threadIdx.x >> 6;
     const int c = blockIdx.x * 64 + cl;
-    float a0 = 0.f, a1 = 0.f;
-    if (c < C) {
-        int r = rg;
-        for (; r + 112 < G; r += 128) {
-            float v[8];
-#pragma unroll
-            for (int k = 0; k < 8; ++k) v[k] = part[(size_t)(r + 16 * k) * C + c];
-            a0 += (v[0] + v[2]) + (v[4] + v[6]);
-            a1 += (v[1] + v[3]) + (v[5] + v[7]);
-        }
-        for (; r < G; r += 16) a0 += part[(size_t)r * C + c];
-    }
-    red[rg][cl] = a0 + a1;
+    red[rg][cl] = c < C ? ia_colsum_rowgroup(part, G, C, c, rg) : 0.f;
     __syncthreads();
     if (rg == 0 && c < C) {
-        float s = 0.f;
-#pragma unroll
-        for (int k = 0; k < 16; ++k) s += red[k][cl];
+        const float s = ia_colsum_16(&red[0][cl], 64);
         if (c < C0) out0[c] = s; else out1[c - C0] = s;
     }
 }
 
 __global__ __launch_bounds__(256) void ia_partials_finish_wide_kernel(const float* __restrict__ part, int G, int64_t C4,
                                                                       int64_t S4, float* __restrict__ out) {
-    for (int64_t i = (int64_t)blockIdx.x * 256 + threadIdx.x; i < C4; i += (int64_t)gridDim.x * 256) {
-        const float4* p = reinterpret_cast<const float4*>(part) + i;
-        float4 a = make_float4(0.f, 0.f, 0.f, 0.f), b = a;
-        int g = 0;
-        for (; g + 1 < G; g += 2) {
-            const float4 x = p[(int64_t)g * S4], y = p[(int64_t)(g + 1) * S4];
-            a.x += x.x; a.y += x.y; a.z += x.z; a.w += x.w;
-            b.x += y.x; b.y += y.y; b.z += y.z; b.w += y.w;
-        }
-        if (g < G) { const float4 x = p[(int64_t)g * S4]; a.x += x.x; a.y += x.y; a.z += x.z; a.w += x.w; }
-        reinterpret_cast<float4*>(out)[i] = make_float4(a.x + b.x, a.y + b.y, a.z + b.z, a.w + b.w);
-    }
+    for (int64_t i = (int64_t)blockIdx.x * 256 + threadIdx.x; i < C4; i += (int64_t)gridDim.x * 256)
+        reinterpret_cast<float4*>(out)[i] = ia_wide_sum4(reinterpret_cast<const float4*>(part) + i, G, S4);
 }
 
 inline void ia_partials_finish_wide_strided(const float* part, int G, int64_t C, int64_t stride, float* out, hipStream_t st) {
```

After: 3678 utterances/s. -2.9%, worse.
